# simonkosina/vbt

Hardware: AMD Instinct MI355X
Metric: frames/sec end-to-end (detect+NMS+track), EfficientDet-Lite0 320x320 (higher is better)
Workload: dtype int8

## Files before the change

### vbt_amd/csrc/band_block.h

```cpp
#pragma once
#include <type_traits>

#include "fused_block.h"

namespace vbt {

#ifndef VBT_BD_WAVES
#define VBT_BD_WAVES 16
#endif
constexpr int BD_WAVES = VBT_BD_WAVES, BD_THREADS = 64 * BD_WAVES;
constexpr int BD_LIT = 3;
constexpr int BD_LIT_NODE = 1;
constexpr int BD_LIT_NODE_WIDE = 3;
constexpr int BD_WP_TAIL = 1024;
constexpr int BD_WD_CHAIN = 12 * 1024 + 512;

#ifdef VBT_BD_PROF
#define BD_STAMP(k) do { if (threadIdx.x == 0) a.prof[(long)blockIdx.x * 8 + (k)] = __builtin_amdgcn_s_memtime(); } while (0)
#else
#define BD_STAMP(k) do { } while (0)
#endif

struct BandArgs {
  const int8_t* x;
  int8_t* out;
  int H, W, Cout, rows, nbands;
  int C, CS;
  int NCG, KS;
  unsigned zx4;
  const v4i* wd;
  const int* bd;
  const float* md;
  Rq rqd;
  const v4i* wp;
  const v4i* wpc;
  const int* bp;
  const float* mp;
  Rq rqp;
  int n_src, chain;
  const int8_t* src[3];
  int sh[3], sw[3], smode[3], spt[3], spl[3];
  AddQ sumq, preq;
#ifdef VBT_BD_PROF
  unsigned long long* prof;
#endif
};

__device__ __forceinline__ unsigned band_source4(const BandArgs& a, int j, long b, int iy, int ix, int cd, bool up2) {
  const int C = a.C;
  const int8_t* sb = a.src[j] + b * (long)a.sh[j] * a.sw[j] * C + 4 * cd;
  if (a.smode[j] == 0) return *(const unsigned*)(sb + (iy * a.sw[j] + ix) * C);
  if (a.smode[j] == 1) {
    int yy, xx;
    if (up2) { yy = iy >> 1; xx = ix >> 1; }
    else { yy = (iy * a.sh[j]) / a.H; xx = (ix * a.sw[j]) / a.W; }
    return *(const unsigned*)(sb + (yy * a.sw[j] + xx) * C);
  }
  unsigned lo = 0u, hi = 0u;
#pragma unroll
  for (int ky = 0; ky < 3; ky++) {
    const int yy = iy * 2 + ky - a.spt[j], yc = min(max(yy, 0), a.sh[j] - 1);
#pragma unroll
    for (int kx = 0; kx < 3; kx++) {
      const int xx = ix * 2 + kx - a.spl[j], xc = min(max(xx, 0), a.sw[j] - 1);
      unsigned t = *(const unsigned*)(sb + (yc * a.sw[j] + xc) * C);
      t = (yy == yc && xx == xc) ? (t ^ 0x80808080u) : 0u;
      lo = pk_max_u16(lo, t & 0x00FF00FFu);
      hi = pk_max_u16(hi, (t >> 8) & 0x00FF00FFu);
    }
  }
  return (lo | (hi << 8)) ^ 0x80808080u;
}

__device__ __forceinline__ uint4 band_source16(const BandArgs& a, int j, long b, int iy, int ix, int sg, bool up2) {
  const int C = a.C;
  const int8_t* sb = a.src[j] + b * (long)a.sh[j] * a.sw[j] * C + 16 * sg;
  if (a.smode[j] == 0) return *(const uint4*)(sb + (iy * a.sw[j] + ix) * C);
  if (a.smode[j] == 1) {
    int yy, xx;
    if (up2) { yy = iy >> 1; xx = ix >> 1; }
    else { yy = (iy * a.sh[j]) / a.H; xx = (ix * a.sw[j]) / a.W; }
    return *(const uint4*)(sb + (yy * a.sw[j] + xx) * C);
  }
  unsigned lo[4] = {0u, 0u, 0u, 0u}, hi[4] = {0u, 0u, 0u, 0u};
#pragma unroll
  for (int ky = 0; ky < 3; ky++) {
    const int yy = iy * 2 + ky - a.spt[j], yc = min(max(yy, 0), a.sh[j] - 1);
#pragma unroll
    for (int kx = 0; kx < 3; kx++) {
      const int xx = ix * 2 + kx - a.spl[j], xc = min(max(xx, 0), a.sw[j] - 1);
      const uint4 t4 = *(const uint4*)(sb + (yc * a.sw[j] + xc) * C);
      const bool in = yy == yc && xx == xc;
      const unsigned tt[4] = {t4.x, t4.y, t4.z, t4.w};
#pragma unroll
      for (int d = 0; d < 4; d++) {
        const unsigned t = in ? (tt[d] ^ 0x80808080u) : 0u;
        lo[d] = pk_max_u16(lo[d], t & 0x00FF00FFu);
        hi[d] = pk_max_u16(hi[d], (t >> 8) & 0x00FF00FFu);
      }
    }
  }
  return make_uint4((lo[0] | (hi[0] << 8)) ^ 0x80808080u, (lo[1] | (hi[1] << 8)) ^ 0x80808080u, (lo[2] | (hi[2] << 8)) ^ 0x80808080u,
                    (lo[3] | (hi[3] << 8)) ^ 0x80808080u);
}

template <int NW, int CT, bool NODES = true, bool CHAIN = false>
__device__ __forceinline__ void sepconv_band_body(const BandArgs& a, int local, unsigned char* bd_smem) {
  constexpr int nwaves = NW, nthreads = 64 * NW;
  static_assert(!CHAIN || CT == 64, "the chained form is built for 64-channel maps");
  constexpr bool C64 = CT == 64, CK = CT != 0;
  constexpr int CS_T = CT == 64 ? 80 : CT;
  static_assert(CT == 0 || CT == 64 || CT == 112, "compile-time widths: 64, 112");
  const long b = fdiv_small(local, frcp(a.nbands));
  const int band = local - (int)b * a.nbands;
  const int tid = threadIdx.x, wave = tid >> 6, lane = tid & 63, r = lane & 15, g = lane >> 4;
  const int y0 = band * a.rows, nr = min(a.rows, a.H - y0);
  const int PW = a.W + 2, NPh = (nr + 2) * PW, NPo = nr * a.W, NPG = (NPo + 15) >> 4;
  const int C = CK ? CT : a.C, CS = CK ? CS_T : a.CS;
  unsigned char* T0 = bd_smem;
  unsigned char* D = T0 + (a.rows + 2) * PW * CS;
  unsigned char* WP = CHAIN ? D : D + (((a.rows * a.W + 15) >> 4) << 4) * CS;
  const int NT = (a.Cout + 15) >> 4, KS = CK ? (CT + 63) / 64 : a.KS, NCG = CK ? (CT + 15) / 16 : a.NCG;
  unsigned char* WB = WP + NT * KS * 1024;
  BD_STAMP(0);

  const v4i* wpg = CHAIN ? a.wpc : a.wp;
  for (int i = tid; i < NT * KS * 64; i += nthreads) *(v4i*)(WP + 16 * i) = wpg[i];
  if constexpr (CHAIN) {
    for (int i = tid; i < 12 * 64; i += nthreads) *(v4i*)(WB + BD_WP_TAIL + 16 * i) = a.wd[i];
    if (tid >= 64 && tid < 80) *(uint4*)(WB + BD_WP_TAIL + 12 * 1024 + 16 * (tid - 64)) = *(const uint4*)((const unsigned char*)a.bd + 16 * (tid - 64));
    else if (tid >= 96 && tid < 112) *(uint4*)(WB + BD_WP_TAIL + 12 * 1024 + 256 + 16 * (tid - 96)) = *(const uint4*)((const unsigned char*)a.md + 16 * (tid - 96));
  }
  if (tid < 4 * NT) *(uint4*)(WB + 16 * tid) = *(const uint4*)((const unsigned char*)a.bp + 16 * tid);
  else if (tid >= 32 && tid < 32 + 4 * NT) *(uint4*)(WB + 512 + 16 * (tid - 32)) = *(const uint4*)((const unsigned char*)a.mp + 16 * (tid - 32));
  const float rcp_pw = frcp(PW);
  if (NODES && a.n_src > 0) {
    const bool up2[3] = {a.H == 2 * a.sh[0] && a.W == 2 * a.sw[0], a.H == 2 * a.sh[1] && a.W == 2 * a.sw[1], a.H == 2 * a.sh[2] && a.W == 2 * a.sw[2]};
    if (CK || (C & 15) == 0) {
      constexpr int LITN = C64 ? BD_LIT_NODE : BD_LIT_NODE_WIDE;
      const int npp = C64 ? 4 : CS >> 4, nreal = C64 ? 4 : C >> 4;
      const float rcp_npp = frcp(npp);
      const int total = NPh * npp;
      for (int i0 = tid; i0 < total; i0 += LITN * nthreads) {
        uint4 us[LITN][3];
        int pofs[LITN];
#pragma unroll
        for (int k = 0; k < LITN; k++) {
          const int i = i0 + k * nthreads, ic = min(i, total - 1);
          const int p = C64 ? ic >> 2 : (CK ? ic / (CS_T >> 4) : fdiv_small(ic, rcp_npp)), sg = ic - p * npp;
          const int hy = fdiv_small(p, rcp_pw), hx = p - hy * PW;
          const int iy = y0 + hy - 1, ix = hx - 1;
          const bool in = i < total && sg < nreal && iy >= 0 && iy < a.H && ix >= 0 && ix < a.W;
          pofs[k] = i < total ? (p * CS + 16 * sg) | (in ? 0 : (1 << 30)) : -1;
#pragma unroll
          for (int j = 0; j < 3; j++) {
            us[k][j] = make_uint4(0u, 0u, 0u, 0u);
            if (j < a.n_src && in) us[k][j] = band_source16(a, j, b, iy, ix, sg, up2[j]);
          }
        }
#pragma unroll
        for (int k = 0; k < LITN; k++) {
          if (pofs[k] < 0) continue;
          uint4 v = make_uint4(a.zx4, a.zx4, a.zx4, a.zx4);
          if (!(pofs[k] >> 30)) {
            const unsigned u0[4] = {us[k][0].x, us[k][0].y, us[k][0].z, us[k][0].w}, u1[4] = {us[k][1].x, us[k][1].y, us[k][1].z, us[k][1].w},
                           u2[4] = {us[k][2].x, us[k][2].y, us[k][2].z, us[k][2].w};
            unsigned o[4];
#pragma unroll
            for (int d = 0; d < 4; d++) {
              if (a.chain == 0) o[d] = addq4(u0[d], u1[d], a.sumq);
              else {
                const unsigned pp = addq4(u0[d], u1[d], a.preq);
                o[d] = a.chain == 1 ? addq4(pp, u2[d], a.sumq) : addq4(u2[d], pp, a.sumq);
              }
            }
            v = make_uint4(o[0], o[1], o[2], o[3]);
          }
          *(uint4*)(T0 + (pofs[k] & 0xFFFFFF)) = v;
        }
      }
    } else {
    const int ndp = CS >> 2, nd = C >> 2;
    const float rcp_ndp = frcp(ndp);
    for (int i = tid; i < NPh * ndp; i += nthreads) {
      const int p = fdiv_small(i, rcp_ndp), cd = i - p * ndp;
      const int hy = fdiv_small(p, rcp_pw), hx = p - hy * PW;
      const int iy = y0 + hy - 1, ix = hx - 1;
      unsigned v = a.zx4;
      if (cd < nd && iy >= 0 && iy < a.H && ix >= 0 && ix < a.W) {
        unsigned us[3] = {0u, 0u, 0u};
#pragma unroll
        for (int j = 0; j < 3; j++)
          if (j < a.n_src) us[j] = band_source4(a, j, b, iy, ix, cd, up2[j]);
        if (a.chain == 0) v = addq4(us[0], us[1], a.sumq);
        else {
          const unsigned pp = addq4(us[0], us[1], a.preq);
          v = a.chain == 1 ? addq4(pp, us[2], a.sumq) : addq4(us[2], pp, a.sumq);
        }
      }
      *(unsigned*)(T0 + p * CS + 4 * cd) = v;
    }
    }
  } else {
    const int8_t* xb = a.x + b * (long)a.H * a.W * C;
    if constexpr (C64) {
      const uint4 z4 = make_uint4(a.zx4, a.zx4, a.zx4, a.zx4);
      const int total = NPh * 4;
      for (int i0 = tid; i0 < total; i0 += BD_LIT * nthreads) {
        uint4 v[BD_LIT];
        int pofs[BD_LIT];
#pragma unroll
        for (int k = 0; k < BD_LIT; k++) {
          const int i = i0 + k * nthreads;
          const int p = i >> 2, sg = i & 3;
          const int hy = fdiv_small(min(p, NPh - 1), rcp_pw), hx = p - hy * PW;
          const int iy = y0 + hy - 1, ix = hx - 1;
          pofs[k] = i < total ? p * 80 + 16 * sg : -1;
          v[k] = z4;
          if (i < total && iy >= 0 && iy < a.H && ix >= 0 && ix < a.W) v[k] = *(const uint4*)(xb + (iy * a.W + ix) * 64 + 16 * sg);
        }
#pragma unroll
        for (int k = 0; k < BD_LIT; k++)
          if (pofs[k] >= 0) *(uint4*)(T0 + pofs[k]) = v[k];
      }
    } else {
    if (CK || (C & 15) == 0) {
      const int npp = CS >> 4, nreal = C >> 4;
      const float rcp_npp = frcp(npp);
      const uint4 z4 = make_uint4(a.zx4, a.zx4, a.zx4, a.zx4);
      const int total = NPh * npp;
      for (int i0 = tid; i0 < total; i0 += BD_LIT * nthreads) {
        uint4 v[BD_LIT];
        int pofs[BD_LIT];
#pragma unroll
        for (int k = 0; k < BD_LIT; k++) {
          const int i = i0 + k * nthreads, ic = min(i, total - 1);
          const int p = CK ? ic / (CS_T >> 4) : fdiv_small(ic, rcp_npp), sg = ic - p * npp;
          const int hy = fdiv_small(p, rcp_pw), hx = p - hy * PW;
          const int iy = y0 + hy - 1, ix = hx - 1;
          pofs[k] = i < total ? p * CS + 16 * sg : -1;
          v[k] = z4;
          if (i < total && sg < nreal && iy >= 0 && iy < a.H && ix >= 0 && ix < a.W) v[k] = *(const uint4*)(xb + (iy * a.W + ix) * C + 16 * sg);
        }
#pragma unroll
        for (int k = 0; k < BD_LIT; k++)
          if (pofs[k] >= 0) *(uint4*)(T0 + pofs[k]) = v[k];
      }
    } else {
    const int ngp = CS >> 3, ng = C >> 3;
    const float rcp_ngp = frcp(ngp);
    const uint2 z2 = make_uint2(a.zx4, a.zx4);
    for (int i = tid; i < NPh * ngp; i += nthreads) {
      const int p = fdiv_small(i, rcp_ngp), sg = i - p * ngp;
      const int hy = fdiv_small(p, rcp_pw), hx = p - hy * PW;
      const int iy = y0 + hy - 1, ix = hx - 1;
      uint2 v = z2;
      if (sg < ng && iy >= 0 && iy < a.H && ix >= 0 && ix < a.W) v = *(const uint2*)(xb + (iy * a.W + ix) * C + 8 * sg);
      *(uint2*)(T0 + p * CS + 8 * sg) = v;
    }
    }
    }
  }
  int tapoff[3];
#pragma unroll
  for (int m = 0; m < 3; m++) {
    const int tap = min(4 * m + g, 8);
    tapoff[m] = ((tap / 3) * PW + (tap % 3)) * CS;
  }
  const float rcp_w = frcp(a.W);
  if constexpr (CHAIN) {
    const unsigned char* WD = WB + BD_WP_TAIL;
    const unsigned char* WDB = WD + 12 * 1024;
    __syncthreads();
    BD_STAMP(1);
    int8_t* ob = a.out + ((b * a.H + y0) * (long)a.W) * a.Cout + 4 * g;
    const bool dword_out = (a.Cout & 3) == 0;
    auto chain = [&](auto fd_c, auto u_c, int pg0) {
      constexpr int U = decltype(u_c)::value, FULL = decltype(fd_c)::value;
      int slot[U];
      const unsigned char* pb[U];
#pragma unroll
      for (int u = 0; u < U; u++) {
        slot[u] = (pg0 + u * nwaves) * 16 + r;
        const int sc = min(slot[u], NPo - 1);
        const int py = fdiv_small(sc, rcp_w);
        pb[u] = T0 + (sc + 2 * py) * CS;
      }
      v4i dv[U];
      {
#pragma unroll
        for (int cg = 0; cg < 4; cg++) {
          v4i wdv[3], bv[U][3], acc[U];
#pragma unroll
          for (int m = 0; m < 3; m++) wdv[m] = *(const v4i*)(WD + ((cg * 3 + m) * 64 + lane) * 16);
          const int4 bq = *(const int4*)(WDB + 64 * cg + 16 * g);
          const float4 mu = *(const float4*)(WDB + 256 + 64 * cg + 16 * g);
#pragma unroll
          for (int u = 0; u < U; u++)
#pragma unroll
            for (int m = 0; m < 3; m++) bv[u][m] = *(const v4i*)(pb[u] + tapoff[m] + 16 * cg);
#pragma unroll
          for (int u = 0; u < U; u++) acc[u] = v4i_from(int4_plus(bq, FULL >= 2 ? RQ_KBIAS : 0));
#pragma unroll
          for (int m = 0; m < 3; m++)
#pragma unroll
            for (int u = 0; u < U; u++) acc[u] = __builtin_amdgcn_mfma_i32_16x16x64_i8(wdv[m], bv[u][m], acc[u], 0, 0, 0);
#pragma unroll
          for (int u = 0; u < U; u++) dv[u][cg] = (int)rq_pack_b<FULL>(acc[u], mu, a.rqd);
          __builtin_amdgcn_sched_barrier(0);
        }
      }
      rq_dispatch(a.rqp, [&](auto fp_c) {
        constexpr int FULL = decltype(fp_c)::value;
        for (int t = 0; t < NT; t++) {
          const int c0 = 16 * t + 4 * g;
          const v4i wv = *(const v4i*)(WP + (t * 64 + lane) * 16);
          const int4 bb = *(const int4*)(WB + 4 * c0);
          const float4 mm = *(const float4*)(WB + 512 + 4 * c0);
          v4i acc[U];
#pragma unroll
          for (int u = 0; u < U; u++) acc[u] = __builtin_amdgcn_mfma_i32_16x16x64_i8(wv, dv[u], v4i_from(int4_plus(bb, FULL >= 2 ? RQ_KBIAS : 0)), 0, 0, 0);
#pragma unroll
          for (int u = 0; u < U; u++) {
            const unsigned d = rq_pack_b<FULL>(acc[u], mm, a.rqp);
            if (slot[u] < NPo && c0 < a.Cout) {
              int8_t* o = ob + (long)slot[u] * a.Cout + 16 * t;
              if (dword_out) *(unsigned*)o = d;
              else
                for (int j = 0; j < 4; j++)
                  if (c0 + j < a.Cout) o[j] = (int8_t)(d >> (8 * j));
            }
          }
        }
      });
    };
    rq_dispatch(a.rqd, [&](auto fd_c) {
      int pg = wave;
      for (; pg + nwaves < NPG; pg += 2 * nwaves) chain(fd_c, std::integral_constant<int, 2>{}, pg);
      if (pg < NPG) chain(fd_c, std::integral_constant<int, 1>{}, pg);
    });
    BD_STAMP(3);
    return;
  }
  const int cg = wave % NCG, sub = wave / NCG, nsub = nwaves / NCG;
  v4i wdv[3];
#pragma unroll
  for (int m = 0; m < 3; m++) wdv[m] = a.wd[(cg * 3 + m) * 64 + lane];
  const int4 bq = *(const int4*)(a.bd + 16 * cg + 4 * g);
  const float4 mu = *(const float4*)(a.md + 16 * cg + 4 * g);
  __syncthreads();
  BD_STAMP(1);
  if (sub < nsub) {
    auto d_units = [&](auto full_c, auto u_c, int pg0) {
      constexpr int U = decltype(u_c)::value, FULL = decltype(full_c)::value;
      const unsigned char* pb[U];
      int slot[U];
#pragma unroll
      for (int u = 0; u < U; u++) {
        slot[u] = (pg0 + u * nsub) * 16 + r;
        const int sc = min(slot[u], NPo - 1);
        const int py = fdiv_small(sc, rcp_w);
        pb[u] = T0 + (sc + 2 * py) * CS + 16 * cg;
      }
      v4i bv[U][3], acc[U];
#pragma unroll
      for (int u = 0; u < U; u++)
#pragma unroll
        for (int m = 0; m < 3; m++) bv[u][m] = *(const v4i*)(pb[u] + tapoff[m]);
#pragma unroll
      for (int u = 0; u < U; u++) acc[u] = v4i_from(int4_plus(bq, FULL >= 2 ? RQ_KBIAS : 0));
#pragma unroll
      for (int m = 0; m < 3; m++)
#pragma unroll
        for (int u = 0; u < U; u++) acc[u] = __builtin_amdgcn_mfma_i32_16x16x64_i8(wdv[m], bv[u][m], acc[u], 0, 0, 0);
#pragma unroll
      for (int u = 0; u < U; u++) *(unsigned*)(D + slot[u] * CS + 16 * cg + 4 * g) = rq_pack_b<FULL>(acc[u], mu, a.rqd);
    };
    auto d_walk = [&](auto full_c) {
      int pg = sub;
      for (; pg + nsub < NPG; pg += 2 * nsub) d_units(full_c, std::integral_constant<int, 2>{}, pg);
      if (pg < NPG) d_units(full_c, std::integral_constant<int, 1>{}, pg);
    };
    rq_dispatch(a.rqd, d_walk);
  }
  __syncthreads();
  BD_STAMP(2);
  const int NU = NPG * NT;
  const float rcp_nt = frcp(NT);
  auto store_unit = [&](int pg, int t, const v4i& acc, const float4& mm) {
    const int slot = pg * 16 + r;
    const int c0 = 16 * t + 4 * g;
    const unsigned d = rq_pack_b(acc, mm, a.rqp);
    if (slot < NPo && c0 < a.Cout) {
      int8_t* o = a.out + ((b * a.H + y0) * (long)a.W + slot) * a.Cout + c0;
      if ((a.Cout & 3) == 0) *(unsigned*)o = d;
      else
        for (int j = 0; j < 4; j++)
          if (c0 + j < a.Cout) o[j] = (int8_t)(d >> (8 * j));
    }
  };
  if (NT == 4 && KS == 1 && a.Cout == 64) {
    const int t = wave & 3, c0 = 16 * t + 4 * g;
    const v4i wv = *(const v4i*)(WP + (t * 64 + lane) * 16);
    const int4 bb = *(const int4*)(WB + 4 * c0);
    const float4 mm = *(const float4*)(WB + 512 + 4 * c0);
    int8_t* ob = a.out + ((b * a.H + y0) * (long)a.W) * a.Cout + c0;
    auto p_units = [&](auto full_c, auto u_c, int pg0) {
      constexpr int U = decltype(u_c)::value, FULL = decltype(full_c)::value;
      v4i dv[U], acc[U];
#pragma unroll
      for (int u = 0; u < U; u++) dv[u] = *(const v4i*)(D + ((pg0 + u * (nwaves / 4)) * 16 + r) * CS + 16 * g);
#pragma unroll
      for (int u = 0; u < U; u++) acc[u] = __builtin_amdgcn_mfma_i32_16x16x64_i8(wv, dv[u], v4i_from(int4_plus(bb, FULL >= 2 ? RQ_KBIAS : 0)), 0, 0, 0);
#pragma unroll
      for (int u = 0; u < U; u++) {
        const int slot = (pg0 + u * (nwaves / 4)) * 16 + r;
        const unsigned d = rq_pack_b<FULL>(acc[u], mm, a.rqp);
        if (slot < NPo) *(unsigned*)(ob + (long)slot * a.Cout) = d;
      }
    };
    auto p_walk = [&](auto full_c) {
      int pg = wave >> 2;
      for (; pg + (nwaves / 4) < NPG; pg += 2 * (nwaves / 4)) p_units(full_c, std::integral_constant<int, 2>{}, pg);
      if (pg < NPG) p_units(full_c, std::integral_constant<int, 1>{}, pg);
    };
    rq_dispatch(a.rqp, p_walk);
  } else if (!C64 && NT <= nwaves && KS <= 2 && (nwaves - NT * (nwaves / NT)) * 8 <= nwaves) {
    const int t = wave % NT, sub = wave / NT, nsub = nwaves / NT;
    if (sub < nsub) {
      const int c0 = 16 * t + 4 * g;
      v4i wv[2];
#pragma unroll
      for (int ks = 0; ks < 2; ks++) wv[ks] = ks < KS ? *(const v4i*)(WP + ((t * KS + ks) * 64 + lane) * 16) : (v4i){0, 0, 0, 0};
      const int4 bb = *(const int4*)(WB + 4 * c0);
      const float4 mm = *(const float4*)(WB + 512 + 4 * c0);
      auto p_units = [&](auto u_c, int pg0) {
        constexpr int U = decltype(u_c)::value;
        v4i dv[U][2], acc[U];
#pragma unroll
        for (int u = 0; u < U; u++)
#pragma unroll
          for (int ks = 0; ks < 2; ks++)
            if (ks < KS) dv[u][ks] = *(const v4i*)(D + ((pg0 + u * nsub) * 16 + r) * CS + 16 * g + 64 * ks);
#pragma unroll
        for (int u = 0; u < U; u++) {
          acc[u] = __builtin_amdgcn_mfma_i32_16x16x64_i8(wv[0], dv[u][0], v4i_from(bb), 0, 0, 0);
          if (KS > 1) acc[u] = __builtin_amdgcn_mfma_i32_16x16x64_i8(wv[1], dv[u][1], acc[u], 0, 0, 0);
        }
#pragma unroll
        for (int u = 0; u < U; u++) store_unit(pg0 + u * nsub, t, acc[u], mm);
      };
      int pg = sub;
      for (; pg + nsub < NPG; pg += 2 * nsub) p_units(std::integral_constant<int, 2>{}, pg);
      if (pg < NPG) p_units(std::integral_constant<int, 1>{}, pg);
    }
  } else {
    for (int u = wave; u < NU; u += nwaves) {
      const int pg = fdiv_small(u, rcp_nt), t = u - pg * NT;
      const int c0 = 16 * t + 4 * g;
      v4i acc = v4i_from(*(const int4*)(WB + 4 * c0));
      const unsigned char* drow = D + (pg * 16 + r) * CS + 16 * g;
      for (int ks = 0; ks < KS; ks++)
        acc = __builtin_amdgcn_mfma_i32_16x16x64_i8(*(const v4i*)(WP + ((t * KS + ks) * 64 + lane) * 16), *(const v4i*)(drow + 64 * ks), acc, 0, 0, 0);
      store_unit(pg, t, acc, *(const float4*)(WB + 512 + 4 * c0));
    }
  }
  BD_STAMP(3);
}

#ifndef VBT_BD_HEAD_WAVES
#define VBT_BD_HEAD_WAVES 8
#endif
#ifndef VBT_BD_HEAD_MAXPX
#define VBT_BD_HEAD_MAXPX 240
#endif
constexpr int BD_HEAD_WAVES = VBT_BD_HEAD_WAVES, BD_HEAD_MAXPX = VBT_BD_HEAD_MAXPX;
constexpr int BD_HEAD_WAVES_WIDE = 16;
#ifdef VBT_DEFINE_BAND_KERNELS
__device__ __forceinline__ int band_problem(const MultiTiles& mt) {
  int pi = 0;
#pragma unroll
  for (int i = 1; i < 12; i++)
    if (i < mt.n && (int)blockIdx.x >= mt.start[i]) pi = i;
  return pi;
}
__global__ __launch_bounds__(64 * BD_HEAD_WAVES) void sepconv_band_kernel(const BandArgs* __restrict__ probs, MultiTiles mt) {
  extern __shared__ __attribute__((aligned(16))) unsigned char bd_smem_dyn[];
  const int pi = band_problem(mt);
  sepconv_band_body<BD_HEAD_WAVES, 64, false>(probs[pi], (int)blockIdx.x - mt.start[pi], bd_smem_dyn);
}
__global__ __launch_bounds__(64 * BD_HEAD_WAVES_WIDE, 2) void sepconv_band_wide_kernel(const BandArgs* __restrict__ probs, MultiTiles mt) {
  extern __shared__ __attribute__((aligned(16))) unsigned char bd_smem_dyn[];
  const int pi = band_problem(mt);
  sepconv_band_body<BD_HEAD_WAVES_WIDE, 0, false>(probs[pi], (int)blockIdx.x - mt.start[pi], bd_smem_dyn);
}
__global__ __launch_bounds__(64 * BD_HEAD_WAVES_WIDE, 2) void sepconv_band_c112_kernel(const BandArgs* __restrict__ probs, MultiTiles mt) {
  extern __shared__ __attribute__((aligned(16))) unsigned char bd_smem_dyn[];
  const int pi = band_problem(mt);
  sepconv_band_body<BD_HEAD_WAVES_WIDE, 112, false>(probs[pi], (int)blockIdx.x - mt.start[pi], bd_smem_dyn);
}
__global__ __launch_bounds__(64 * BD_HEAD_WAVES) __attribute__((amdgpu_waves_per_eu(6))) void sepconv_band_chain_kernel(const BandArgs* __restrict__ probs, MultiTiles mt) {
  extern __shared__ __attribute__((aligned(16))) unsigned char bd_smem_dyn[];
  const int pi = band_problem(mt);
  sepconv_band_body<BD_HEAD_WAVES, 64, false, true>(probs[pi], (int)blockIdx.x - mt.start[pi], bd_smem_dyn);
}
__global__ __launch_bounds__(BD_THREADS) void sepconv_band_one_kernel(BandArgs a) {
  extern __shared__ __attribute__((aligned(16))) unsigned char bd_smem_dyn[];
  sepconv_band_body<BD_WAVES, 64>(a, (int)blockIdx.x, bd_smem_dyn);
}
__global__ __launch_bounds__(BD_THREADS) void sepconv_band_one_chain_kernel(BandArgs a) {
  extern __shared__ __attribute__((aligned(16))) unsigned char bd_smem_dyn[];
  sepconv_band_body<BD_WAVES, 64, true, true>(a, (int)blockIdx.x, bd_smem_dyn);
}
__global__ __launch_bounds__(BD_THREADS) void sepconv_band_one_wide_kernel(BandArgs a) {
  extern __shared__ __attribute__((aligned(16))) unsigned char bd_smem_dyn[];
  sepconv_band_body<BD_WAVES, 0>(a, (int)blockIdx.x, bd_smem_dyn);
}
__global__ __launch_bounds__(BD_THREADS) void sepconv_band_one_c112_kernel(BandArgs a) {
  extern __shared__ __attribute__((aligned(16))) unsigned char bd_smem_dyn[];
  sepconv_band_body<BD_WAVES, 112>(a, (int)blockIdx.x, bd_smem_dyn);
}
#endif

}
```

### vbt_amd/csrc/dev_common.h

```cpp
#pragma once
#include "common.h"

namespace vbt {

typedef int v4i __attribute__((ext_vector_type(4)));

__device__ __forceinline__ int requant(int acc, float mult, int zp, int lo, int hi) {
  float t = (float)acc * mult;
  t = fminf(fmaxf(t, -65536.0f), 65536.0f);
  int q = (int)__builtin_rintf(t) + zp;
  return min(max(q, lo), hi);
}
__device__ __forceinline__ unsigned pack4(int a, int b, int c, int d) {
  return (unsigned)(a & 255) | ((unsigned)(b & 255) << 8) | ((unsigned)(c & 255) << 16) | ((unsigned)(d & 255) << 24);
}

struct Rq {
  float lo_f, hi_f, off;
  int full;
  int kb;
};
constexpr int RQ_KBIAS = 0x4B400000;
__host__ __device__ inline Rq make_rq(int zp, int lo, int hi, int kb = 0) {
  return Rq{(float)(lo - zp), (float)(hi - zp), (float)(zp + 128), (lo <= -128 && hi >= 127) ? 1 : 0, kb};
}
__device__ __forceinline__ float rq_u8(float accf, float mult, const Rq& q) {
  float r = __builtin_rintf(accf * mult);
  return __builtin_amdgcn_fmed3f(r, q.lo_f, q.hi_f) + q.off;
}
__device__ __forceinline__ unsigned pack4_u8f(float a, float b, float c, float d) {
  unsigned v = __builtin_amdgcn_cvt_pk_u8_f32(a, 0, 0);
  v = __builtin_amdgcn_cvt_pk_u8_f32(b, 1, v);
  v = __builtin_amdgcn_cvt_pk_u8_f32(c, 2, v);
  v = __builtin_amdgcn_cvt_pk_u8_f32(d, 3, v);
  return v ^ 0x80808080u;
}
typedef float v2f __attribute__((ext_vector_type(2)));
template <int FULLK = -1>
__device__ __forceinline__ unsigned rq_pack_b(const v4i& acc, const float4& mu, const Rq& q) {
  v2f f0, f1;
  if (FULLK >= 2) {
    const v2f kf = {12582912.0f, 12582912.0f};
    f0 = (v2f){__int_as_float(acc[0]), __int_as_float(acc[1])} - kf;
    f1 = (v2f){__int_as_float(acc[2]), __int_as_float(acc[3])} - kf;
  } else {
    f0 = (v2f){(float)acc[0], (float)acc[1]};
    f1 = (v2f){(float)acc[2], (float)acc[3]};
  }
  v2f t0 = f0 * (v2f){mu.x, mu.y};
  v2f t1 = f1 * (v2f){mu.z, mu.w};
  const v2f off = {q.off, q.off};
  if ((FULLK >= 0 && (FULLK & 1)) || (FULLK < 0 && q.full)) {
    const v2f magic = {12582912.0f, 12582912.0f};
    const v2f back = {q.off - 12582912.0f, q.off - 12582912.0f};
    v2f r0 = (t0 + magic) + back;
    v2f r1 = (t1 + magic) + back;
    return pack4_u8f(r0.x, r0.y, r1.x, r1.y);
  }
  v2f r0 = {__builtin_amdgcn_fmed3f(__builtin_rintf(t0.x), q.lo_f, q.hi_f), __builtin_amdgcn_fmed3f(__builtin_rintf(t0.y), q.lo_f, q.hi_f)};
  v2f r1 = {__builtin_amdgcn_fmed3f(__builtin_rintf(t1.x), q.lo_f, q.hi_f), __builtin_amdgcn_fmed3f(__builtin_rintf(t1.y), q.lo_f, q.hi_f)};
  r0 = r0 + off;
  r1 = r1 + off;
  return pack4_u8f(r0.x, r0.y, r1.x, r1.y);
}
__device__ __forceinline__ v4i diag_operand(unsigned wb, int i) {
  const unsigned sh = wb << (8 * (i & 3));
  const int d = i >> 2;
  return (v4i){d == 0 ? (int)sh : 0, d == 1 ? (int)sh : 0, d == 2 ? (int)sh : 0, d == 3 ? (int)sh : 0};
}
__device__ __forceinline__ v4i toeplitz_operand(unsigned w4, int c) {
  const int sh = 8 * c;
  return (v4i){(int)((w4 & 0xffu) << sh), (int)(((w4 >> 8) & 0xffu) << sh), (int)(((w4 >> 16) & 0xffu) << sh), (int)((w4 >> 24) << sh)};
}
__device__ __forceinline__ int fdiv_small(int n, float rcp_d) { return (int)(((float)n + 0.5f) * rcp_d); }
__device__ __forceinline__ float frcp(int d) { return __builtin_amdgcn_rcpf((float)d); }
__device__ __forceinline__ v4i v4i_from(const int4& b) { return (v4i){b.x, b.y, b.z, b.w}; }
__device__ __forceinline__ int4 int4_plus(const int4& b, int k) { return make_int4(b.x + k, b.y + k, b.z + k, b.w + k); }
template <class F>
__device__ __forceinline__ void rq_dispatch(const Rq& q, F&& f) {
  if (q.kb) { if (q.full) f(std::integral_constant<int, 3>{}); else f(std::integral_constant<int, 2>{}); }
  else { if (q.full) f(std::integral_constant<int, 1>{}); else f(std::integral_constant<int, 0>{}); }
}

__device__ __forceinline__ unsigned rq_pack_i(const v4i& acc, const int4& b, const float4& mu, const Rq& q) {
  const v4i a2 = {acc[0] + b.x, acc[1] + b.y, acc[2] + b.z, acc[3] + b.w};
  return rq_pack_b(a2, mu, q);
}

struct AddQ { int bias, am, bm, shift, lo, hi, off; };
static inline AddQ make_addq(const AddParams& p, int z_out, int lo, int hi) {
  return AddQ{p.bias, p.am, p.bm, p.shift, lo - z_out, hi - z_out, z_out + 128};
}
__device__ __forceinline__ int addq_u8(int a, int b, const AddQ& q) {
  const int t = (q.bias + __mul24(a, q.am) + __mul24(b, q.bm)) >> q.shift;
  return min(max(t, q.lo), q.hi) + q.off;
}
__device__ __forceinline__ unsigned addq4(unsigned ua, unsigned ub, const AddQ& q) {
  unsigned r = 0;
#pragma unroll
  for (int e = 0; e < 4; e++)
    r |= (unsigned)addq_u8((int)(int8_t)(ua >> (8 * e)), (int)(int8_t)(ub >> (8 * e)), q) << (8 * e);
  return r ^ 0x80808080u;
}

__device__ __forceinline__ unsigned max4_s8(unsigned a, unsigned b) {
  unsigned r = 0;
#pragma unroll
  for (int j = 0; j < 4; j++) {
    int x = (int)(int8_t)(a >> (8 * j)), y = (int)(int8_t)(b >> (8 * j));
    r |= (unsigned)(max(x, y) & 255) << (8 * j);
  }
  return r;
}

struct Epi {
  const int* bias;
  const float* mult;
  int zp, lo, hi;
  Rq rq;
};

__device__ __forceinline__ void store_tile(const v4i acc[4], const Epi& e, int8_t* __restrict__ out, long m, int N,
                                           int nb, int g) {
  int c0 = nb * 64 + 16 * g;
  if (c0 >= N) return;
  unsigned d[4];
#pragma unroll
  for (int t = 0; t < 4; t++) {
    int4 b = *(const int4*)(e.bias + c0 + 4 * t);
    float4 mu = *(const float4*)(e.mult + c0 + 4 * t);
    d[t] = rq_pack_i(acc[t], b, mu, e.rq);
  }
  int8_t* o = out + m * N + c0;
  if ((N & 15) == 0) {
    *(uint4*)o = make_uint4(d[0], d[1], d[2], d[3]);
  } else if ((N & 3) == 0) {
#pragma unroll
    for (int t = 0; t < 4; t++)
      if (c0 + 4 * t < N) *(unsigned*)(o + 4 * t) = d[t];
  } else {
#pragma unroll
    for (int t = 0; t < 4; t++)
#pragma unroll
      for (int j = 0; j < 4; j++)
        if (c0 + 4 * t + j < N) o[4 * t + j] = (int8_t)(d[t] >> (8 * j));
  }
}

}
```

### vbt_amd/csrc/fused_block.h

```cpp
#pragma once
#include "tpz_geom.h"
#include "halo_geom.h"
#include "fused_params_geom.h"
#include "dev_common.h"

namespace vbt {

struct FusedArgs {
  const int8_t* x;
  int8_t* out;
  int H, W, Cin, OH, OW, Cout;
  int pad_t, pad_l;
  int TX, TY, tiles_x, tiles_y;
  int T0S;
  int nchunks;
  int zx;
  const long* we;
  const int* be;
  const float* me;
  int KSe, ze, loe, hie;
  Rq rqe;
  const long* we3;
  const long* wdm3;
  const v4i* wp3;
  int nch3, KSp3;
  const float* wd;
  const int* bd;
  const float* md;
  int zd, lod, hid;
  Rq rqd;
  const long* wdm;
  const int* bdm;
  const v4i* wd64;
  const long* wd64c;
  const unsigned* wtz;
  const v4i* wp;
  const v4i* wpt;
  const v4i* wpt3;
  const int* bp;
  const float* mp;
  int KSp, zo, lop, hip;
  Rq rqp;
  const unsigned char* cpar;
  int has_res;
  AddQ resq;
  int n_src;
  const int8_t* src[3];
  int sh[3], sw[3], smode[3], spt[3], spl[3];
  int chain;
  AddQ sumq, preq;
};

__device__ __forceinline__ unsigned node_sum4(const unsigned u[3], const FusedArgs& a) {
  if (a.chain == 0) return addq4(u[0], u[1], a.sumq);
  const unsigned p = addq4(u[0], u[1], a.preq);
  return a.chain == 1 ? addq4(p, u[2], a.sumq) : addq4(u[2], p, a.sumq);
}

typedef unsigned short v2u16 __attribute__((ext_vector_type(2)));
__device__ __forceinline__ unsigned pk_max_u16(unsigned a, unsigned b) {
  v2u16 x, y;
  __builtin_memcpy(&x, &a, 4);
  __builtin_memcpy(&y, &b, 4);
  v2u16 r = __builtin_elementwise_max(x, y);
  unsigned o;
  __builtin_memcpy(&o, &r, 4);
  return o;
}

constexpr int FB_EST = 80;
constexpr int FB_DST = 80;

template <int NP> struct ParamPieces { v4i v[NP > 0 ? (NP + 255) / 256 : 1]; };
template <int NP> __device__ __forceinline__ void pp_fetch(ParamPieces<NP>& r, const unsigned char* src, int tid) {
#pragma unroll
  for (int i = 0; i < (NP + 255) / 256; i++) r.v[i] = *(const v4i*)(src + 16 * min(tid + 256 * i, NP - 1));
}
template <int NP> __device__ __forceinline__ void pp_store(const ParamPieces<NP>& r, unsigned char* dst, int tid) {
#pragma unroll
  for (int i = 0; i < (NP + 255) / 256; i++)
    if (256 * i + 255 < NP || tid + 256 * i < NP) *(v4i*)(dst + 16 * (tid + 256 * i)) = r.v[i];
}
template <int KK, int S, int NBP, bool EXPAND, bool MDW, int KSE = 0, int NT = 4, int PPW = 1, bool DW64 = false, bool TPZ = false, int NTL = 0, bool PLDS = false>
__device__ __forceinline__ void fused_block_body(const FusedArgs& a, int tile, unsigned char* fb_smem) {
  static_assert(PPW == 1 || MDW, "128-pixel tiles exist for the matrix-pipe depthwise only");
  static_assert(NTL >= 0 && NTL <= 4 && (NTL == 0 || EXPAND), "a tile-major last block (MBConv only) holds one to four tiles");
  constexpr int NBW = NTL ? NBP - 1 : NBP;
  static_assert(!DW64 || (EXPAND && MDW && (KK == 3 || KK == 5)), "DW64: fused expand blocks, 3x3 / 5x5");
  static_assert(!TPZ || (DW64 && (S == 1 || S == 2) && (NT == 3 || NT == 4) && NBP <= 2 && (KSE == 1 || KSE == 2)), "TPZ: a form of DW64");
  constexpr TpzGeom TG = TPZ ? tpz_geom(KK, S, PPW, NT) : TpzGeom{};
  constexpr int KT2 = (S * (S - 1) + KK + 1) / 2;
  static_assert(!PLDS || (EXPAND && MDW && (KSE == 1 || KSE == 2)), "PLDS: MBConv tiles with register-resident expand weights and no early depthwise request");
  constexpr FusedParamsGeom PG = fused_params_geom(NT, KSE > 0 ? KSE : 1, TPZ ? FPF_TOEPLITZ : DW64 ? FPF_DIAG64 : FPF_MATRIX, KK, S, NBP, NTL);
  constexpr int NPE = PLDS ? PG.pe / 16 : 0, NPD = PLDS ? PG.pd / 16 : 0, NPP = PLDS ? PG.pp / 16 : 0, NPB = PLDS ? PG.pb / 16 : 0;
  const int tid = threadIdx.x, wave = __builtin_amdgcn_readfirstlane(tid >> 6), lane = tid & 63, r = lane & 15, g = lane >> 4;
  const int trow = fdiv_small(tile, frcp(a.tiles_x));
  const int tx = tile - trow * a.tiles_x;
  const int bimg = fdiv_small(trow, frcp(a.tiles_y));
  const int ty = trow - bimg * a.tiles_y;
  const long b = bimg;
  const int oy0 = ty * a.TY, ox0 = tx * a.TX;
  const int TXp = (a.TX + 3) & ~3;
  const int HWx = (TXp - 1) * S + KK, HWy = (a.TY - 1) * S + KK, NPh = HWx * HWy;
  const int iy0 = oy0 * S - a.pad_t, ix0 = ox0 * S - a.pad_l;
  const float rcp_hwx = frcp(HWx), rcp_txp = frcp(TXp);
  unsigned char* T0 = fb_smem;
  unsigned char* E = T0 + ((NPh * a.T0S + 15) & ~15);
  constexpr int EST = (EXPAND && NT == 3) ? (DW64 ? 48 : 72) : FB_EST;
  unsigned char* D = E + (EXPAND ? (TPZ ? TG.e_bytes : ((NPh * EST + 15) & ~15)) : 0);
  bool stage_p = false;
  if constexpr (!EXPAND && NBP <= 2) stage_p = a.nchunks == 1;
  unsigned char* WPS = D + 64 * PPW * FB_DST;
  unsigned char* BPS = WPS + NBP * 4096;
  unsigned char* const PAe = D + 64 * PPW * FB_DST + (TPZ ? 8 * TG.DSK : 0);
  unsigned char* const PAd = PAe + PG.pe;
  unsigned char* const PAp = PAd + PG.pd;
  unsigned char* const PAb = PAp + PG.pp;
  constexpr int CH = 16 * NT;
  const int nch = NT == 3 ? a.nch3 : a.nchunks;
  ParamPieces<NPE> rpe;
  ParamPieces<NPD> rpd;
  ParamPieces<NPP> rpp;
  ParamPieces<NPB> rpb;
  if constexpr (PLDS) {
    pp_fetch(rpe, a.cpar, tid);
    pp_fetch(rpd, a.cpar + PG.pe, tid);
    pp_fetch(rpp, a.cpar + PG.pe + PG.pd, tid);
    pp_fetch(rpb, a.cpar + (long)nch * PG.chunk, tid);
  }

  bool summed = false;
  if constexpr (!EXPAND) summed = a.n_src > 0;
  if (summed) {
    const int nd = a.Cin >> 2;
    const unsigned zb4 = (unsigned)(a.zx & 255) * 0x01010101u;
    const int pstep = fdiv_small(256, frcp(nd));
    int p = fdiv_small(tid, frcp(nd));
    const int cd = tid - p * nd;
    const bool up2[3] = {a.H == 2 * a.sh[0] && a.W == 2 * a.sw[0], a.H == 2 * a.sh[1] && a.W == 2 * a.sw[1], a.H == 2 * a.sh[2] && a.W == 2 * a.sw[2]};
    for (; tid < pstep * nd && p < NPh; p += pstep) {
      const int hy = fdiv_small(p, rcp_hwx), hx = p - hy * HWx;
      const int iy = iy0 + hy, ix = ix0 + hx;
      unsigned v = zb4;
      if (!halo_outside(iy, ix, a.H, a.W)) {
        unsigned us[3] = {0u, 0u, 0u};
#pragma unroll
        for (int j = 0; j < 3; j++) {
          if (j < a.n_src) {
            const int8_t* sb = a.src[j] + b * (long)a.sh[j] * a.sw[j] * a.Cin + 4 * cd;
            unsigned u;
            if (a.smode[j] == 0) {
              u = *(const unsigned*)(sb + ((long)iy * a.sw[j] + ix) * a.Cin);
            } else if (a.smode[j] == 1) {
              int yy, xx;
              if (up2[j]) { yy = iy >> 1; xx = ix >> 1; }
              else { yy = (iy * a.sh[j]) / a.H; xx = (ix * a.sw[j]) / a.W; }
              u = *(const unsigned*)(sb + ((long)yy * a.sw[j] + xx) * a.Cin);
            } else {
              unsigned tv[9];
#pragma unroll
              for (int ky = 0; ky < 3; ky++) {
                const int yy = iy * 2 + ky - a.spt[j];
                const int yc = min(max(yy, 0), a.sh[j] - 1);
#pragma unroll
                for (int kx = 0; kx < 3; kx++) {
                  const int xx = ix * 2 + kx - a.spl[j];
                  const int xc = min(max(xx, 0), a.sw[j] - 1);
                  const unsigned t = *(const unsigned*)(sb + ((long)yc * a.sw[j] + xc) * a.Cin);
                  tv[ky * 3 + kx] = (yy == yc && xx == xc) ? (t ^ 0x80808080u) : 0u;
                }
              }
              unsigned lo = 0u, hi = 0u;
#pragma unroll
              for (int q = 0; q < 9; q++) {
                const unsigned l = tv[q] & 0x00FF00FFu, h = (tv[q] >> 8) & 0x00FF00FFu;
                lo = pk_max_u16(lo, l);
                hi = pk_max_u16(hi, h);
              }
              u = (lo | (hi << 8)) ^ 0x80808080u;
            }
            us[j] = u;
          }
        }
        v = node_sum4(us, a);
      }
      *(unsigned*)(T0 + p * a.T0S + 4 * cd) = v;
    }
  } else {
    if ((a.Cin & 15) == 0) {
      const int ng = a.Cin >> 4;
      const unsigned zb1 = (unsigned)(a.zx & 255) * 0x01010101u;
      const uint4 zb = make_uint4(zb1, zb1, zb1, zb1);
      const int8_t* xb = a.x + b * (long)a.H * a.W * a.Cin;
      const int pstep = fdiv_small(256, frcp(ng));
      int p = fdiv_small(tid, frcp(ng));
      const int sg = tid - p * ng;
      for (; tid < pstep * ng && p < NPh; p += pstep) {
        const int hy = fdiv_small(p, rcp_hwx), hx = p - hy * HWx;
        const int iy = iy0 + hy, ix = ix0 + hx;
        uint4 v = zb;
        if (!halo_outside(iy, ix, a.H, a.W)) v = *(const uint4*)(xb + (iy * a.W + ix) * a.Cin + 16 * sg);
        unsigned char* dst = T0 + p * a.T0S + 16 * sg;
        if constexpr (EXPAND) {
          *(uint2*)dst = make_uint2(v.x, v.y);
          *(uint2*)(dst + 8) = make_uint2(v.z, v.w);
        } else {
          *(uint4*)dst = v;
        }
      }
    } else {
    const int ng = a.Cin >> 3;
    const unsigned long long zb = (unsigned long long)(a.zx & 255) * 0x0101010101010101ull;
    const int8_t* xb = a.x + b * (long)a.H * a.W * a.Cin;
    const int pstep = fdiv_small(256, frcp(ng));
    int p = fdiv_small(tid, frcp(ng));
    const int sg = tid - p * ng;
    for (; tid < pstep * ng && p < NPh; p += pstep) {
      const int hy = fdiv_small(p, rcp_hwx), hx = p - hy * HWx;
      const int iy = iy0 + hy, ix = ix0 + hx;
      unsigned long long v = zb;
      if (!halo_outside(iy, ix, a.H, a.W)) v = *(const unsigned long long*)(xb + (iy * a.W + ix) * a.Cin + 8 * sg);
      *(unsigned long long*)(T0 + p * a.T0S + 8 * sg) = v;
    }
    }
  }
  if (stage_p) {
    for (int i = tid; i < NBP * 256; i += 256) *(uint4*)(WPS + 16 * i) = *(const uint4*)((const unsigned char*)a.wp + 16 * (long)i);
    if (tid < NBP * 16) *(uint4*)(BPS + 16 * tid) = *(const uint4*)((const unsigned char*)a.bp + 16 * tid);
    else if (tid < NBP * 32) *(uint4*)(BPS + 16 * tid) = *(const uint4*)((const unsigned char*)a.mp + 16 * (tid - NBP * 16));
  }
  const int NPG = (NPh + 15) >> 4;
  unsigned oob_mask = 0;
  const bool border = EXPAND && halo_border(iy0, ix0, HWx, HWy, a.H, a.W);
  if (border) oob_mask = halo_oob_mask(wave, r, NPh, HWx, iy0, ix0, a.H, a.W, [&](int p) { return fdiv_small(p, rcp_hwx); });
  v4i acc[PPW][NBP][4];
#pragma unroll
  for (int pp = 0; pp < PPW; pp++)
#pragma unroll
    for (int nb = 0; nb < NBP; nb++)
#pragma unroll
      for (int t = 0; t < 4; t++) acc[pp][nb][t] = (v4i){0, 0, 0, 0};
  const int cq = tid & 15, strip = tid >> 4;
  const int nsx = TXp >> 2;
  const int sy = fdiv_small(strip, frcp(nsx)), sx = (strip - sy * nsx) * 4;
  const bool dw_active = sy < a.TY;
  int hbase[4 * PPW];
#pragma unroll
  for (int pg = 0; pg < 4 * PPW; pg++) hbase[pg] = 0;
  if constexpr (MDW && !DW64) {
#pragma unroll
    for (int pg = 0; pg < 4 * PPW; pg++) {
      int slot = pg * 16 + r;
      int sq = TXp == 8 ? (slot >> 3) : fdiv_small(slot, rcp_txp);
      int py_ = min(sq, a.TY - 1), px_ = slot - sq * TXp;
      hbase[pg] = (py_ * S) * HWx + px_ * S;
    }
  }
  const int wq0 = TPZ ? wave * NT : 0;
  int tz_e = 0, tz_d = 0;
  if constexpr (TPZ) {
    tz_e = tpz_e_offset(TG, S, r, g, wq0);
    tz_d = tpz_d_offset(TG, S, PPW, FB_DST, r, g, wq0);
  }
  constexpr int KTP = (KK * KK + 1) / 2;
  long wpre[KTP];
  int4 bpre = make_int4(0, 0, 0, 0);
  float4 mpre = make_float4(0.f, 0.f, 0.f, 0.f);
  if constexpr (!EXPAND && MDW) {
    const long* wm0 = a.wdm + ((long)wave * KTP) * 64 + lane;
#pragma unroll
    for (int mi = 0; mi < KTP; mi++) wpre[mi] = wm0[mi * 64];
    bpre = *(const int4*)(a.bdm + 16 * wave + 4 * g);
    mpre = *(const float4*)(a.md + 16 * wave + 4 * g);
  }
  if constexpr (PLDS) {
    pp_store(rpe, PAe, tid);
    pp_store(rpd, PAd, tid);
    pp_store(rpp, PAp, tid);
    pp_store(rpb, PAb, tid);
  }
  __syncthreads();

  const long* const wdm_ = NT == 3 ? a.wdm3 : a.wdm;
  for (int c = 0; c < nch; c++) {
    constexpr bool PREF_DW = EXPAND && MDW && KSE >= 3;
    if constexpr (PREF_DW) {
      if (NT == 4 || wave < NT) {
        const long* wmc = wdm_ + ((long)(c * NT + wave) * KTP) * 64 + lane;
#pragma unroll
        for (int mi = 0; mi < KTP; mi++) wpre[mi] = wmc[mi * 64];
        bpre = *(const int4*)(a.bdm + c * CH + 16 * wave + 4 * g);
        mpre = *(const float4*)(a.md + c * CH + 16 * wave + 4 * g);
      }
    }
    unsigned wtz[TPZ ? NT * KT2 : 1];
    if constexpr (TPZ && !PLDS) {
      const unsigned* wt = a.wtz + ((long)(c * 4 * NT + wq0) * KT2) * 64 + lane;
#pragma unroll
      for (int i = 0; i < NT * KT2; i++) wtz[i] = wt[i * 64];
    }
    const unsigned char* const cnext = PLDS ? a.cpar + (long)min(c + 1, nch - 1) * PG.chunk : nullptr;
    if (EXPAND) {
      int4 eb[NT];
      float4 em[NT];
      const unsigned zeb = (unsigned)(a.ze & 255) * 0x01010101u;
      const long* w = (NT == 3 ? a.we3 : a.we) + (long)c * a.KSe * NT * 64 + lane;
      long wreg[KSE > 0 ? KSE : 1][NT];
      if constexpr (PLDS) {
        pp_fetch(rpe, cnext, tid);
#pragma unroll
        for (int t = 0; t < NT; t++) {
          eb[t] = *(const int4*)(PAe + PG.o_be + 4 * (4 * NT * g + 4 * t));
          em[t] = *(const float4*)(PAe + PG.o_me + 4 * (4 * NT * g + 4 * t));
        }
#pragma unroll
        for (int ks = 0; ks < KSE; ks++)
#pragma unroll
          for (int t = 0; t < NT; t++) wreg[ks][t] = *(const long*)(PAe + 8 * ((ks * NT + t) * 64 + lane));
      } else {
#pragma unroll
      for (int t = 0; t < NT; t++) {
        eb[t] = *(const int4*)(a.be + c * CH + 4 * NT * g + 4 * t);
        em[t] = *(const float4*)(a.me + c * CH + 4 * NT * g + 4 * t);
      }
      if constexpr (KSE > 0) {
#pragma unroll
        for (int ks = 0; ks < KSE; ks++)
#pragma unroll
          for (int t = 0; t < NT; t++) wreg[ks][t] = w[(ks * NT + t) * 64];
      }
      }
      auto expand_loop = [&](auto full_tag, auto oob_tag) {
        constexpr int FULLK = decltype(full_tag)::value;
        constexpr bool OOB = decltype(oob_tag)::value;
        int4 ebk[NT];
#pragma unroll
        for (int t = 0; t < NT; t++) ebk[t] = int4_plus(eb[t], FULLK >= 2 ? RQ_KBIAS : 0);
        for (int i = 0, pg = wave; pg < NPG; pg += 4, i++) {
          const int p = pg * 16 + r;
          v4i ea[NT];
#pragma unroll
          for (int t = 0; t < NT; t++) ea[t] = v4i_from(ebk[t]);
          const unsigned char* brow = T0 + (__umul24((unsigned)min(p, NPh - 1), (unsigned)a.T0S) + 8u * g);
          if constexpr (KSE > 0) {
#pragma unroll
            for (int ks = 0; ks < KSE; ks++) {
              long bv = *(const long*)(brow + 32 * ks);
#pragma unroll
              for (int t = 0; t < NT; t++) ea[t] = __builtin_amdgcn_mfma_i32_16x16x32_i8(wreg[ks][t], bv, ea[t], 0, 0, 0);
            }
          } else {
#pragma unroll 2
            for (int ks = 0; ks < a.KSe; ks++) {
              long bv = *(const long*)(brow + 32 * ks);
#pragma unroll
              for (int t = 0; t < NT; t++) ea[t] = __builtin_amdgcn_mfma_i32_16x16x32_i8(w[(ks * NT + t) * 64], bv, ea[t], 0, 0, 0);
            }
          }
          unsigned d[NT];
#pragma unroll
          for (int t = 0; t < NT; t++) {
            d[t] = rq_pack_b<FULLK>(ea[t], em[t], a.rqe);
            if constexpr (OOB)
              if ((oob_mask >> i) & 1u) d[t] = zeb;
          }
          if (p < NPh) {
            if constexpr (TPZ) {
              const int hy = fdiv_small(p, rcp_hwx), hx = p - hy * HWx;
              unsigned char* ep = E + tpz_e_store(TG, hy, hx, NT * g);
#pragma unroll
              for (int t = 0; t < NT; t++) *(unsigned*)(ep + t * TG.EQS) = d[t];
            } else if constexpr (NT == 4) {
              *(uint4*)(E + p * FB_EST + 16 * g) = make_uint4(d[0], d[1], d[2], d[3]);
            } else {
#pragma unroll
              for (int t = 0; t < NT; t++) *(unsigned*)(E + p * EST + 4 * NT * g + 4 * t) = d[t];
            }
          }
        }
      };
      if (border) rq_dispatch(a.rqe, [&](auto full_tag) { expand_loop(full_tag, std::true_type{}); });
      else rq_dispatch(a.rqe, [&](auto full_tag) { expand_loop(full_tag, std::false_type{}); });
      __syncthreads();
      if constexpr (PLDS) {
        pp_store(rpe, PAe, tid);
        if (c > 0) pp_store(rpp, PAp, tid);
        pp_fetch(rpd, cnext + PG.pe, tid);
      }
    }
    if constexpr (TPZ) {
      constexpr int NU = NT * PPW, PGE = tpz_e_group(TG, S), PGD = tpz_d_group(TG, PPW, FB_DST);
      int4 bq[NT];
      float4 mq[NT];
      if constexpr (!PLDS) {
#pragma unroll
        for (int q = 0; q < NT; q++) {
          bq[q] = *(const int4*)(a.bdm + c * CH + 4 * (wq0 + q));
          mq[q] = *(const float4*)(a.md + c * CH + 4 * (wq0 + q));
        }
      }
      const unsigned char* const tzw = PAd + 4 * (wq0 * KT2 * 64 + lane);
      const unsigned char* const tzb = PAd + 16 * wq0;
      auto tz_bias = [&](int q) { if constexpr (PLDS) return *(const int4*)(tzb + PG.o_bd + 16 * q); else return bq[q]; };
      auto tz_mult = [&](int q) { if constexpr (PLDS) return *(const float4*)(tzb + PG.o_md + 16 * q); else return mq[q]; };
      auto tz_tap = [&](int i) { if constexpr (PLDS) return *(const unsigned*)(tzw + 256 * i); else return wtz[i]; };
      const unsigned char* eb = E + tz_e;
      unsigned char* db = D + tz_d;
      auto tz_walk = [&](auto mode_tag) {
        constexpr int RM = decltype(mode_tag)::value;
#pragma unroll
        for (int u0 = 0; u0 < NU; u0 += 2) {
          v4i dq[2];
#pragma unroll
          for (int u = 0; u < 2; u++) dq[u] = v4i_from(int4_plus(tz_bias((u0 + u < NU ? u0 + u : u0) / PPW), RM >= 2 ? RQ_KBIAS : 0));
#pragma unroll
          for (int mi = 0; mi < KT2; mi++)
#pragma unroll
            for (int u = 0; u < 2; u++) {
              if (u0 + u >= NU) continue;
              const int q = (u0 + u) / PPW, pg = (u0 + u) % PPW;
              const v4i bv = *(const v4i*)(eb + q * TG.EQS + pg * PGE + mi * 2 * TG.EYS);
              dq[u] = __builtin_amdgcn_mfma_i32_16x16x64_i8(toeplitz_operand(tz_tap(q * KT2 + mi), r & 3), bv, dq[u], 0, 0, 0);
            }
#pragma unroll
          for (int u = 0; u < 2; u++) {
            if (u0 + u >= NU) continue;
            const int q = (u0 + u) / PPW, pg = (u0 + u) % PPW;
            *(unsigned*)(db + pg * PGD + 4 * q) = rq_pack_b<RM>(dq[u], tz_mult(q), a.rqd);
          }
        }
      };
      rq_dispatch(a.rqd, tz_walk);
    } else if constexpr (DW64) {
      constexpr int TXP = 8 * PPW, HWX = (TXP - 1) * S + KK;
      constexpr int KT64 = KK == 3 ? 3 : 7;
      constexpr int PGS = (16 / TXP) * S * HWX * EST;
      if (NT == 4 || wave < NT) {
        const unsigned long long wc = PLDS ? *(const unsigned long long*)(PAd + 8 * (wave * 64 + lane)) : (unsigned long long)a.wd64c[(long)(c * NT + wave) * 64 + lane];
        v4i wreg[KT64];
#pragma unroll
        for (int mi = 0; mi < KT64; mi++) wreg[mi] = diag_operand((unsigned)(wc >> (8 * mi)) & 0xffu, r);
        const int4 bq0 = PLDS ? *(const int4*)(PAd + PG.o_bd + 4 * (16 * wave + 4 * g)) : *(const int4*)(a.bdm + c * CH + 16 * wave + 4 * g);
        const float4 mum = PLDS ? *(const float4*)(PAd + PG.o_md + 4 * (16 * wave + 4 * g)) : *(const float4*)(a.md + c * CH + 16 * wave + 4 * g);
        const int hb = TXP == 8 ? ((r >> 3) * S * HWX + (r & 7) * S) : r * S;
        const unsigned char* baseH = E + hb * EST + 16 * wave + g * EST;
        const unsigned char* baseV = E + hb * EST + 16 * wave + g * (HWX * EST);
        auto dw_walk = [&](auto mode_tag) {
          constexpr int RM = decltype(mode_tag)::value;
          const int4 bqm = int4_plus(bq0, RM >= 2 ? RQ_KBIAS : 0);
#pragma unroll
          for (int pg = 0; pg < 4 * PPW; pg += 2) {
            v4i dqa = v4i_from(bqm), dqb = v4i_from(bqm);
#pragma unroll
            for (int mi = 0; mi < KT64; mi++) {
              const unsigned char* bp = (KK == 5 && mi == 5) ? baseV : baseH;
              const int off = KK == 3 ? mi * HWX * EST : (mi < 5 ? mi * HWX * EST : (mi == 5 ? 4 * EST : (4 * HWX + 4) * EST));
              const v4i bva = *(const v4i*)(bp + pg * PGS + off);
              const v4i bvb = *(const v4i*)(bp + (pg + 1) * PGS + off);
              dqa = __builtin_amdgcn_mfma_i32_16x16x64_i8(wreg[mi], bva, dqa, 0, 0, 0);
              dqb = __builtin_amdgcn_mfma_i32_16x16x64_i8(wreg[mi], bvb, dqb, 0, 0, 0);
            }
            *(unsigned*)(D + (pg * 16 + r) * FB_DST + 16 * wave + 4 * g) = rq_pack_b<RM>(dqa, mum, a.rqd);
            *(unsigned*)(D + ((pg + 1) * 16 + r) * FB_DST + 16 * wave + 4 * g) = rq_pack_b<RM>(dqb, mum, a.rqd);
          }
        };
        rq_dispatch(a.rqd, dw_walk);
      }
    } else if constexpr (MDW) {
      constexpr int KT = (KK * KK + 1) / 2;
      const unsigned char* Ein = EXPAND ? E : T0 + 64 * c;
      const int est = EXPAND ? EST : a.T0S;
// ... 349 lines not shown
```

### vbt_amd/csrc/k_postprocess.hip

```cpp
#include "launchers.h"

namespace vbt {

constexpr int POST_CAP = 2048;
#ifdef VBT_POST_PROF
__device__ unsigned long long g_post_prof[16];
#define POST_STAMP(i) do { if (threadIdx.x == 0 && blockIdx.x == 0) { const unsigned long long t_ = __builtin_amdgcn_s_memtime(); atomicAdd(&g_post_prof[i], t_ - t_last); t_last = t_; } } while (0)
#else
#define POST_STAMP(i) do { } while (0)
#endif

constexpr int POST_THREADS = 1024;
constexpr int POST_FAST = 1024;
constexpr int POST_LDS_FIXED = 32768 + 1024 + 1024 + 2048 + 2048 + 256 + 32 * 16 + 128 + 128;
static_assert(POST_CAP * 4 + POST_FAST * 4 + POST_FAST * 16 + POST_FAST * 4 <= 32768, "keys | sorted keys | boxes | scores share the histogram's 32 KB");
int post_lds_bytes(int A) { return ((A + 15) & ~15) + POST_LDS_FIXED; }

__device__ __forceinline__ int wave_incl_scan_i(int x) {
  x += __builtin_amdgcn_update_dpp(0, x, 0x111, 0xf, 0xf, false);
  x += __builtin_amdgcn_update_dpp(0, x, 0x112, 0xf, 0xf, false);
  x += __builtin_amdgcn_update_dpp(0, x, 0x114, 0xf, 0xf, false);
  x += __builtin_amdgcn_update_dpp(0, x, 0x118, 0xf, 0xf, false);
  x += __builtin_amdgcn_update_dpp(0, x, 0x142, 0xa, 0xf, false);
  x += __builtin_amdgcn_update_dpp(0, x, 0x143, 0xc, 0xf, false);
  return x;
}
__device__ __forceinline__ int wave_first_lane(bool flag) {
  const unsigned long long m = __ballot(flag);
  return m ? __ffsll((long long)m) - 1 : 64;
}

__global__ __launch_bounds__(POST_THREADS) void postprocess_kernel(PostArgs p, float* __restrict__ boxes, float* __restrict__ scores,
                                                                   float* __restrict__ classes, int* __restrict__ counts) {
  extern __shared__ __attribute__((aligned(16))) unsigned char post_smem[];
  constexpr int NT = POST_THREADS;
  const int tid = threadIdx.x, lane = tid & 63, wave = tid >> 6;
  const long b = blockIdx.x;
#ifdef VBT_POST_PROF
  unsigned long long t_last = __builtin_amdgcn_s_memtime();
#endif
  const int A = p.A;
  int* hist32 = (int*)post_smem;
  unsigned* keys = (unsigned*)hist32;
  unsigned* skeys = keys + POST_CAP;
  float4* lbox = (float4*)(skeys + POST_FAST);
  float* lsc = (float*)(lbox + POST_FAST);
  int* rhist = (int*)(post_smem + 32768);
  float* s_score = (float*)(rhist + 256);
  double* s_dq = (double*)(s_score + 256);
  double* s_ex = s_dq + 256;
  signed char* s_rank = (signed char*)(s_ex + 256);
  float4* selbox = (float4*)(s_rank + 256);
  int* sv = (int*)(selbox + 32);
  unsigned char* cb = post_smem + POST_LDS_FIXED;
  int& s_n = sv[0]; int& s_qlo = sv[1]; int& s_qhi = sv[2]; int& s_i0 = sv[3]; int& s_i1 = sv[4]; int& s_nsel = sv[5]; int& s_done = sv[6];
  int& s_blo = sv[7]; int& s_bhi = sv[8];
  int* s_wtot = sv + 12;
  constexpr int PS = 5;
  const int n4 = (A + 3) >> 2;
  const int b1 = p.base[1], b2 = p.base[2], b3 = p.base[3], b4 = p.base[4];
  auto level_of = [&](int a) -> int { return (a >= b1) + (a >= b2) + (a >= b3) + (a >= b4); };
  const unsigned char *pc0, *pb0;
  long ce1, ce2, ce3, ce4, be1, be2, be3, be4;
  {
    auto cbias = [&](int l) { return (long)p.cls[l] + (b * (long)(p.base[l + 1] - p.base[l]) - p.base[l]) * (long)p.C; };
    auto bbias = [&](int l) { return (long)p.box[l] + (b * (long)(p.base[l + 1] - p.base[l]) - p.base[l]) * 4; };
    pc0 = (const unsigned char*)cbias(0); pb0 = (const unsigned char*)bbias(0);
    ce1 = cbias(1) - cbias(0); ce2 = cbias(2) - cbias(1); ce3 = cbias(3) - cbias(2); ce4 = cbias(4) - cbias(3);
    be1 = bbias(1) - bbias(0); be2 = bbias(2) - bbias(1); be3 = bbias(3) - bbias(2); be4 = bbias(4) - bbias(3);
  }
  auto cls_ptr = [&](int a) -> const unsigned char* {
    long o = (long)a * p.C;
    o += a >= b1 ? ce1 : 0l; o += a >= b2 ? ce2 : 0l; o += a >= b3 ? ce3 : 0l; o += a >= b4 ? ce4 : 0l;
    return pc0 + o;
  };
  auto box_ptr = [&](int a) -> const unsigned char* {
    long o = 4l * a;
    o += a >= b1 ? be1 : 0l; o += a >= b2 ? be2 : 0l; o += a >= b3 ? be3 : 0l; o += a >= b4 ? be4 : 0l;
    return pb0 + o;
  };
  auto whole = [&](int i, const unsigned char* src) -> bool {
    const int a = 4 * i;
    return level_of(a) == level_of(a + 3) && a + 3 < A && (((unsigned long)src) & 3ul) == 0;
  };
  auto patch = [&](int i) -> unsigned {
    unsigned w = 0;
    for (int e = 0; e < 4; e++)
      if (4 * i + e < A) w |= (unsigned)*cls_ptr(4 * i + e) << (8 * e);
    return w;
  };
  if (p.C == 1) {
    unsigned w[PS];
#pragma unroll
    for (int k = 0; k < PS; k++)
      w[k] = *(const unsigned*)((unsigned long)cls_ptr(4 * min(tid + NT * k, n4 - 1)) & ~3ul);
#pragma unroll
    for (int k = 0; k < PS; k++)
      if (tid + NT * k < n4) ((unsigned*)cb)[tid + NT * k] = w[k];
#pragma unroll 1
    for (int i = tid + NT * PS; i < n4; i += NT) ((unsigned*)cb)[i] = *(const unsigned*)((unsigned long)cls_ptr(4 * i) & ~3ul);
#pragma unroll 1
    for (int i = tid; i < n4; i += NT)
      if (!whole(i, cls_ptr(4 * i))) ((unsigned*)cb)[i] = patch(i);
  } else {
    auto best4 = [&](int i) -> unsigned {
      unsigned w = 0;
#pragma unroll
      for (int e = 0; e < 4; e++) {
        const int a = min(4 * i + e, A - 1);
        const signed char* src = (const signed char*)cls_ptr(a);
        int best = src[0];
        for (int c = 1; c < p.C; c++) best = max(best, (int)src[c]);
        w |= ((unsigned)best & 255u) << (8 * e);
      }
      return w;
    };
    if (p.C == 2) {
      constexpr unsigned HB = 0x80808080u;
      auto pair_max = [&](uint2 v) -> unsigned {
        const unsigned w0 = v.x ^ HB, w1 = v.y ^ HB;
        const unsigned m0 = pk_max_u16(w0 & 0x00FF00FFu, (w0 >> 8) & 0x00FF00FFu);
        const unsigned m1 = pk_max_u16(w1 & 0x00FF00FFu, (w1 >> 8) & 0x00FF00FFu);
        return ((m0 & 0xFFu) | ((m0 >> 8) & 0xFF00u) | ((m1 & 0xFFu) << 16) | ((m1 << 8) & 0xFF000000u)) ^ HB;
      };
      auto whole2 = [&](int i, const unsigned char* src) -> bool {
        const int a = 4 * i;
        return level_of(a) == level_of(a + 3) && a + 3 < A && (((unsigned long)src) & 7ul) == 0;
      };
      uint2 w[PS];
#pragma unroll
      for (int k = 0; k < PS; k++)
        w[k] = *(const uint2*)((unsigned long)cls_ptr(4 * min(tid + NT * k, n4 - 1)) & ~7ul);
#pragma unroll
      for (int k = 0; k < PS; k++)
        if (tid + NT * k < n4) ((unsigned*)cb)[tid + NT * k] = pair_max(w[k]);
#pragma unroll 1
      for (int i = tid + NT * PS; i < n4; i += NT) ((unsigned*)cb)[i] = pair_max(*(const uint2*)((unsigned long)cls_ptr(4 * i) & ~7ul));
#pragma unroll 1
      for (int i = tid; i < n4; i += NT)
        if (!whole2(i, cls_ptr(4 * i))) ((unsigned*)cb)[i] = best4(i);
    } else {
#pragma unroll 1
      for (int i = tid; i < n4; i += NT) ((unsigned*)cb)[i] = best4(i);
    }
  }
#pragma unroll
  for (int k = 0; k < 8; k++) hist32[tid + NT * k] = 0;
  if (tid < 256) {
    rhist[tid] = 0;
    s_score[tid] = ((const float*)p.tables)[tid];
    s_dq[tid] = ((const double*)(p.tables + 1024))[tid];
    s_ex[tid] = ((const double*)(p.tables + 3072))[tid];
    s_rank[tid] = ((const signed char*)(p.tables + 5120))[tid];
  }
  if (tid == 0) { s_nsel = 0; s_done = 0; }
  __syncthreads();
  POST_STAMP(0);
  unsigned u[PS];
#pragma unroll
  for (int k = 0; k < PS; k++) u[k] = ((const unsigned*)cb)[min(tid + NT * k, n4 - 1)] ^ 0x80808080u;
  {
    const int copy = tid & 31;
#pragma unroll
    for (int k = 0; k < PS; k++) {
      const int i = tid + NT * k;
#pragma unroll
      for (int e = 0; e < 4; e++)
        if (4 * i + e < A) atomicAdd(&hist32[(((u[k] >> (8 * e)) & 255u) << 5) + copy], 1);
    }
    for (int i = tid + NT * PS; i < n4; i += NT) {
      const unsigned w = ((const unsigned*)cb)[i] ^ 0x80808080u;
#pragma unroll
      for (int e = 0; e < 4; e++)
        if (4 * i + e < A) atomicAdd(&hist32[(((w >> (8 * e)) & 255u) << 5) + copy], 1);
    }
  }
  __syncthreads();
  {
    const int bin = tid >> 2, part = tid & 3;
    int c = 0;
#pragma unroll
    for (int k = 0; k < 8; k++) c += hist32[(bin << 5) + 8 * part + ((k + bin) & 7)];
    if (c) atomicAdd(&rhist[(int)s_rank[bin] + 128], c);
  }
  __syncthreads();
  POST_STAMP(1);
  int qcur = 127;
  int seg0 = 0;
  while (true) {
    if (wave == 0) {
      int v[4], before[4];
      int sum = 0;
#pragma unroll
      for (int j = 0; j < 4; j++) {
        const int r = 127 - (4 * lane + j);
        v[j] = (r <= qcur && r >= p.qmin) ? rhist[r + 128] : 0;
        before[j] = sum;
        sum += v[j];
      }
      const int excl = wave_incl_scan_i(sum) - sum;
      int ffail = 4, ftop = 4;
#pragma unroll
      for (int j = 3; j >= 0; j--) {
        const int r = 127 - (4 * lane + j);
        const int bf = excl + before[j];
        const bool ok = r > qcur || (r >= p.qmin && bf < 256 && bf + v[j] <= POST_CAP);
        if (!ok) ffail = j;
        if (v[j] > 0) ftop = j;
      }
      const int lf = wave_first_lane(ffail < 4), lt = wave_first_lane(ftop < 4);
      const int tfail = lf < 64 ? 4 * lf + __builtin_amdgcn_readlane(ffail, lf) : 256;
      const int ttop = lt < 64 ? 4 * lt + __builtin_amdgcn_readlane(ftop, lt) : 256;
      if (lane == 0) {
        if (ttop >= 256) {
          s_done = 1;
        } else if (tfail <= ttop) {
          s_qhi = 127 - ttop; s_qlo = 127 - ttop; s_i0 = seg0; s_i1 = min(seg0 + POST_CAP, A);
        } else {
          s_qhi = 127 - ttop; s_qlo = 128 - tfail; s_i0 = 0; s_i1 = A;
        }
        s_blo = 255; s_bhi = 0;
      }
    }
    __syncthreads();
    POST_STAMP(2);
    if (s_done) break;
    const int qhi = s_qhi, qlo = s_qlo, i0 = s_i0, i1 = s_i1;
    if (tid < 256) {
      const int r = (int)s_rank[tid];
      const unsigned long long m = __ballot(r >= qlo && r <= qhi);
      if (lane == 0 && m) {
        atomicMin(&s_blo, 64 * wave + __ffsll((long long)m) - 1);
        atomicMax(&s_bhi, 64 * wave + 63 - __clzll((long long)m));
      }
    }
    __syncthreads();
    POST_STAMP(11);
    {
      constexpr unsigned H = 0x80808080u;
      const unsigned LO7 = ((unsigned)s_blo * 0x01010101u) & ~H, NLO = ~((unsigned)s_blo * 0x01010101u);
      const unsigned SP = (unsigned)(s_bhi - s_blo) * 0x01010101u;
      const bool fullrange = i0 == 0 && i1 == A;
      auto hits = [&](unsigned x, int i) -> unsigned {
        const unsigned d = ((x | H) - LO7) ^ ((x ^ NLO) & H);
        const unsigned t = (SP | H) - (d & ~H);
        unsigned m = ((SP & ~d) | (~(SP ^ d) & t)) & H;
        if (fullrange) {
          if (i == n4 - 1 && (A & 3)) m &= (1u << (8 * (A & 3))) - 1u;
        } else {
          const int lo = min(max(i0 - 4 * i, 0), 4), hi = min(max(i1 - 4 * i, 0), 4);
          m &= (unsigned)(((1ull << (8 * hi)) - 1ull) & ~((1ull << (8 * lo)) - 1ull));
        }
        return m;
      };
      unsigned hm[PS];
      int cnt = 0;
#pragma unroll
      for (int k = 0; k < PS; k++) {
        hm[k] = tid + NT * k < n4 ? hits(u[k], tid + NT * k) : 0u;
        cnt += __popc(hm[k]);
      }
#pragma unroll 1
      for (int i = tid + NT * PS; i < n4; i += NT) cnt += __popc(hits(((const unsigned*)cb)[i] ^ H, i));
      const int incl = wave_incl_scan_i(cnt);
      if (lane == 63) s_wtot[wave] = incl;
      __syncthreads();
      POST_STAMP(12);
      int pos = incl - cnt;
#pragma unroll
      for (int w = 0; w < NT / 64; w++) pos += (w < wave) ? s_wtot[w] : 0;
      if (tid == NT - 1) s_n = pos + cnt;
      auto emit = [&](unsigned x, unsigned m, int i) {
#pragma unroll 1
        while (m) {
          const int e = (__ffs((int)m) - 1) >> 3;
          m &= m - 1u;
          keys[pos++] = ((unsigned)(127 - (int)s_rank[(x >> (8 * e)) & 255u]) << 16) | (unsigned)(4 * i + e);
        }
      };
#pragma unroll
      for (int k = 0; k < PS; k++)
        if (hm[k]) emit(u[k], hm[k], tid + NT * k);
#pragma unroll 1
      for (int i = tid + NT * PS; i < n4; i += NT) {
        const unsigned x = ((const unsigned*)cb)[i] ^ H;
        const unsigned m = hits(x, i);
        if (m) emit(x, m, i);
      }
    }
    __syncthreads();
    const int n = s_n;
    const bool fast = n <= POST_FAST;
    const unsigned* sk = fast ? skeys : keys;
    if (fast) {
      const int nq = (n + 3) >> 2;
      if (tid < 4 * nq - n) keys[n + tid] = 0xFFFFFFFFu;
    } else {
      int n2 = 2048;
      for (int i = n + tid; i < n2; i += NT) keys[i] = 0xFFFFFFFFu;
    }
    __syncthreads();
    POST_STAMP(3);
    if (fast) {
      const int nq = (n + 3) >> 2;
      const int parts = n > 0 ? min(NT / n, 4) : 1;
      int* partial = (int*)lbox;
      if (tid < parts * n) {
        const int m = tid % n, part = tid / n;
        const unsigned mine = keys[m];
        int r = 0;
#pragma unroll 4
        for (int j = part * nq / parts; j < (part + 1) * nq / parts; j++) {
          const uint4 k4 = ((const uint4*)keys)[j];
          r += (k4.x < mine) + (k4.y < mine) + (k4.z < mine) + (k4.w < mine);
        }
        partial[part * POST_FAST + m] = r;
      }
      __syncthreads();
      if (tid < n) {
        int r = partial[tid];
        for (int q = 1; q < parts; q++) r += partial[q * POST_FAST + tid];
        skeys[r] = keys[tid];
      }
      __syncthreads();
    } else {
      const int n2 = 2048;
      for (int k = 2; k <= n2; k <<= 1)
        for (int j = k >> 1; j > 0; j >>= 1) {
          for (int i = tid; i < n2; i += NT) {
            int ixj = i ^ j;
            if (ixj > i) {
              unsigned a = keys[i], c = keys[ixj];
              bool up = (i & k) == 0;
              if ((a > c) == up) { keys[i] = c; keys[ixj] = a; }
            }
          }
          __syncthreads();
        }
    }
    POST_STAMP(4);
#ifdef VBT_POST_PROF
    if (tid == 0 && blockIdx.x == 0) { atomicAdd(&g_post_prof[8], 1ull); atomicAdd(&g_post_prof[9], (unsigned long long)n); }
#endif
    auto decode = [&](unsigned key, float& sc) -> float4 {
      const int a = (int)(key & 0xFFFFu);
      const int q = 127 - (int)(key >> 16);
      const unsigned bq = *(const unsigned*)box_ptr(a);
      const float4 an = *(const float4*)(p.anchors + (long)a * 4);
      const float yc = (float)(s_dq[(int)((bq & 255u) ^ 128u)] * (double)an.z + (double)an.x);
      const float xc = (float)(s_dq[(int)(((bq >> 8) & 255u) ^ 128u)] * (double)an.w + (double)an.y);
      const float hh = (float)(0.5 * s_ex[(int)(((bq >> 16) & 255u) ^ 128u)] * (double)an.z);
      const float hw = (float)(0.5 * s_ex[(int)((bq >> 24) ^ 128u)] * (double)an.w);
      sc = s_score[q + 128];
      return make_float4(yc - hh, xc - hw, yc + hh, xc + hw);
    };
    if (fast) {
      if (tid < n) {
        float sc;
        lbox[tid] = decode(skeys[tid], sc);
        lsc[tid] = sc;
      }
      __syncthreads();
    }
    POST_STAMP(13);
    if (wave == 0) {
      float* selarea = (float*)(sv + 32);
      auto sup = [&](float4 sb, float sa, float4 cx, float ca) -> bool {
        const float iy0 = fmaxf(sb.x, cx.x), ix0 = fmaxf(sb.y, cx.y);
        const float iy1 = fminf(sb.z, cx.z), ix1 = fminf(sb.w, cx.w);
        const float inter = fmaxf(iy1 - iy0, 0.0f) * fmaxf(ix1 - ix0, 0.0f);
        return sa > 0.0f && ca > 0.0f && inter / (sa + ca - inter) > p.iou_thr;
      };
      int nsel = s_nsel;
      for (int base = 0; base < n && nsel < p.max_det; base += 64) {
        int ci = base + lane;
        bool alive = ci < n;
        float4 bx = make_float4(0.f, 0.f, 0.f, 0.f);
        float sc = 0.f;
        int anchor = 0;
        if (alive) {
          anchor = (int)(sk[ci] & 0xFFFFu);
          if (fast) { bx = lbox[ci]; sc = lsc[ci]; }
          else bx = decode(sk[ci], sc);
        }
        const float area = (bx.z - bx.x) * (bx.w - bx.y);
        if (alive)
          for (int s = 0; s < nsel; s++)
            if (sup(selbox[s], selarea[s], bx, area)) { alive = false; break; }
        while (nsel < p.max_det) {
          const unsigned long long mask = __ballot(alive);
          if (mask == 0ull) break;
          const int j = __ffsll((long long)mask) - 1;
          float4 sb;
          sb.x = __int_as_float(__builtin_amdgcn_readlane(__float_as_int(bx.x), j));
          sb.y = __int_as_float(__builtin_amdgcn_readlane(__float_as_int(bx.y), j));
          sb.z = __int_as_float(__builtin_amdgcn_readlane(__float_as_int(bx.z), j));
          sb.w = __int_as_float(__builtin_amdgcn_readlane(__float_as_int(bx.w), j));
          const float ss = __int_as_float(__builtin_amdgcn_readlane(__float_as_int(sc), j));
          const float sa = __int_as_float(__builtin_amdgcn_readlane(__float_as_int(area), j));
          const int sel_anchor = __builtin_amdgcn_readlane(anchor, j);
          if (lane == 0) {
            selbox[nsel] = sb;
            selarea[nsel] = sa;
            float* bo = boxes + (b * p.max_det + nsel) * 4;
            bo[0] = sb.x; bo[1] = sb.y; bo[2] = sb.z; bo[3] = sb.w;
            scores[b * p.max_det + nsel] = ss;
            int cls_id = 0;
            if (p.C > 1) {
              const unsigned char* src = cls_ptr(sel_anchor);
              int best = -128;
              for (int c = 0; c < p.C; c++) {
                const int r = (int)s_rank[(int)(src[c] ^ 128u)];
                if (r > best) { best = r; cls_id = c; }
              }
            }
            classes[b * p.max_det + nsel] = (float)cls_id;
          }
          __threadfence_block();
          nsel++;
          if (lane == j) alive = false;
          else if (alive && sup(sb, sa, bx, area)) alive = false;
        }
      }
      if (lane == 0) s_nsel = nsel;
    }
    __syncthreads();
    POST_STAMP(5);
    if (s_nsel >= p.max_det) break;
    if (qhi == qlo && rhist[qhi + 128] > POST_CAP && i1 < A) { seg0 = i1; qcur = qhi; }
    else { seg0 = 0; qcur = qlo - 1; }
    __syncthreads();
  }
  const int nsel = s_nsel;
  for (int s = nsel + tid; s < p.max_det; s += NT) {
    float* bo = boxes + (b * p.max_det + s) * 4;
    bo[0] = bo[1] = bo[2] = bo[3] = 0.0f;
    scores[b * p.max_det + s] = 0.0f;
    classes[b * p.max_det + s] = 0.0f;
  }
  if (tid == 0) counts[b] = nsel;
  POST_STAMP(6);
#ifdef VBT_POST_PROF
  if (tid == 0 && blockIdx.x == 0) atomicAdd(&g_post_prof[10], 1ull);
#endif
}

int launch_postprocess(const PostArgs& p, int lds_bytes, int B, float* boxes, float* scores, float* classes, int* counts, hipStream_t st) {
  if (lds_bytes > 64 * 1024) VBT_LDS_OPT_IN(postprocess_kernel);
  postprocess_kernel<<<dim3((unsigned)B), POST_THREADS, lds_bytes, st>>>(p, boxes, scores, classes, counts);
  return VBT_OK;
}

}

#ifdef VBT_POST_PROF
extern "C" int vbt_post_prof_read(unsigned long long* out16, int reset) {
  if (reset) { unsigned long long z[16] = {0}; VBT_HIP_CHECK(hipMemcpyToSymbol(HIP_SYMBOL(vbt::g_post_prof), z, sizeof(z))); return VBT_OK; }
  VBT_HIP_CHECK(hipDeviceSynchronize());
  VBT_HIP_CHECK(hipMemcpyFromSymbol(out16, HIP_SYMBOL(vbt::g_post_prof), 16 * sizeof(unsigned long long)));
  return VBT_OK;
}
#endif
```

### vbt_amd/csrc/plan_geom.h

```cpp
#pragma once
#include <algorithm>

#include "launchers.h"

namespace vbt {

inline void choose_tile(int OH, int OW, int KK, int S, bool expand, int* TXo, int* TYo, int slots = 64) {
  double best = 1e300;
  for (int TX = 1; TX <= std::min(OW, 64); TX++) {
    int TXp = (TX + 3) & ~3;
    int TY = std::min(OH, slots / TXp);
    if (TY < 1) continue;
    int tiles = ((OW + TX - 1) / TX) * ((OH + TY - 1) / TY);
    int NPh = ((TXp - 1) * S + KK) * ((TY - 1) * S + KK);
    double cost = tiles * ((expand ? 1.0 : 0.35) * NPh + (double)slots);
    if (cost < best) { best = cost; *TXo = TX; *TYo = TY; }
  }
}

inline int fused_tile_lds(const FusedArgs& a, int k, int stride, int TX, int TY, int est, int ppw, int nbp, int e_bytes = -1) {
  const int TXp = (TX + 3) & ~3;
  const int NPh = ((TXp - 1) * stride + k) * ((TY - 1) * stride + k);
  int lds = ((NPh * a.T0S + 15) & ~15) + (e_bytes >= 0 ? e_bytes : ((NPh * est + 15) & ~15)) + ppw * 64 * FB_DST;
  if (!est && a.nchunks == 1 && nbp <= 2) lds += nbp * (4096 + 512);
  return lds;
}

inline int band_lds(const BandArgs& a, bool chained = false) {
  const int NT = (a.Cout + 15) / 16;
  const int t0 = (a.rows + 2) * (a.W + 2) * a.CS, wp = NT * a.KS * 1024 + BD_WP_TAIL;
  return chained ? t0 + wp + BD_WD_CHAIN : t0 + (((a.rows * a.W + 15) >> 4) << 4) * a.CS + wp;
}

}
```

### vbt_amd/csrc/planner.hip

```cpp
#include <algorithm>
#include <cmath>
#include <cstdlib>
#include <functional>
#include <initializer_list>

#include "detector_model.h"
using vbt::v4i;
#include "weight_pack.h"

namespace vbt {

static int conv_kb(const vbt_model* m, const OpRec& op) {
  const bool off = getenv("VBT_NO_KBIAS") != nullptr;
  if (off || (op.type != OP_STEM && op.type != OP_PW && op.type != OP_DW)) return 0;
  const TensorRec& tin = m->tensors[op.inputs[0]];
  const TensorRec& tout = m->tensors[op.output];
  const int8_t* w = (const int8_t*)(m->blob.data() + op.w_off);
  const int32_t* bq = (const int32_t*)(m->blob.data() + op.b_off);
  const bool dw = op.type == OP_DW;
  const int N = tout.c, K = dw ? op.k * op.k : op.k * op.k * tin.c;
  for (int co = 0; co < N; co++) {
    long long sa = 0;
    for (int k = 0; k < K; k++) sa += std::abs((int)(dw ? w[(size_t)k * N + co] : w[(size_t)co * K + k]));
    if (255 * sa + std::llabs((long long)bq[co]) >= (1ll << 22) - 1) return 0;
  }
  return 1;
}


struct NodeSrc { int n = 0; int tensor[3]; int mode[3]; int rs_op[3] = {-1, -1, -1}; int pre_add = -1; int chain = 0; };

static Cost cost_of(const vbt_model* m, std::initializer_list<int> ops, const NodeSrc* ns = nullptr) {
  Cost c;
  for (int oi : ops)
    if (oi >= 0) c += m->op_steps[oi].cost;
  if (ns) c += cost_of(m, {ns->rs_op[0], ns->rs_op[1], ns->rs_op[2], ns->pre_add});
  return c;
}

template <typename Args>
static void fill_node_sources(Args& a, const NodeSrc& ns, const vbt_model* m, int sum_op) {
  a.n_src = ns.n;
  for (int j = 0; j < ns.n; j++) {
    const TensorRec& ts = m->tensors[ns.tensor[j]];
    a.sh[j] = ts.h; a.sw[j] = ts.w; a.smode[j] = ns.mode[j];
    if (ns.mode[j] == 2) { a.spt[j] = m->ops[ns.rs_op[j]].pad_t; a.spl[j] = m->ops[ns.rs_op[j]].pad_l; }
  }
  a.sumq = m->op_steps[sum_op].addq;
  a.chain = 0;
  if (ns.pre_add >= 0) {
    a.chain = ns.chain;
    a.preq = m->op_steps[ns.pre_add].addq;
  }
}

static int make_image_bundle(vbt_model* m, int e_op, int d_op, int p_op, int KSe, ImageBundle* out) {
  const OpRec &eop = m->ops[e_op], &dop = m->ops[d_op], &pop = m->ops[p_op];
  const TensorRec &tin = m->tensors[eop.inputs[0]], &tdin = m->tensors[dop.inputs[0]], &tout = m->tensors[pop.output];
  const int8_t* we = (const int8_t*)(m->blob.data() + eop.w_off);
  const int8_t* wd = (const int8_t*)(m->blob.data() + dop.w_off);
  const int8_t* wpj = (const int8_t*)(m->blob.data() + pop.w_off);
  const int Ce = tdin.c, Cp = (Ce + 63) / 64 * 64, kk = dop.k * dop.k, NB = (tout.c + 63) / 64, nch = Cp / 64;
  std::vector<long> pe, pp;
  pack_weights(we, Ce, tin.c, KSe, nch, nullptr, pe);
  pack_weights(wpj, tout.c, Ce, Cp / 32, NB, nullptr, pp);
  const std::vector<int> be = fold_bias((const int32_t*)(m->blob.data() + eop.b_off), we, Ce, tin.c, tin.zero_point, W_ROWS, Cp);
  const std::vector<int> bd = fold_bias((const int32_t*)(m->blob.data() + dop.b_off), wd, Ce, kk, tdin.zero_point, W_TAPS, Cp);
  const std::vector<float> me = pad_floats((const float*)(m->blob.data() + eop.m_off), Ce, Cp);
  const std::vector<float> md = pad_floats((const float*)(m->blob.data() + dop.m_off), Ce, Cp);
  ImageBundle ib;
  ib.o_be = KSe * 2048; ib.o_me = ib.o_be + 256; ib.o_dw = ib.o_me + 256;
  ib.o_bd = ib.o_dw + ((kk * 64 + 15) & ~15); ib.o_md = ib.o_bd + 256; ib.o_wp = ib.o_md + 256;
  ib.bytes = ib.o_wp + NB * 4096;
  std::vector<unsigned char> rec((size_t)nch * ib.bytes, 0);
  for (int c = 0; c < nch; c++) {
    unsigned char* R = rec.data() + (size_t)c * ib.bytes;
    memcpy(R, pe.data() + (size_t)c * KSe * 4 * 64, (size_t)KSe * 2048);
    memcpy(R + ib.o_be, &be[64 * c], 256);
    memcpy(R + ib.o_me, &me[64 * c], 256);
    memcpy(R + ib.o_bd, &bd[64 * c], 256);
    memcpy(R + ib.o_md, &md[64 * c], 256);
    for (int t = 0; t < kk; t++)
      for (int i = 0; i < 64 && 64 * c + i < Ce; i++) R[ib.o_dw + t * 64 + i] = (unsigned char)wd[(size_t)t * Ce + 64 * c + i];
    for (int nb = 0; nb < NB; nb++)
      for (int k2 = 0; k2 < 2; k2++)
        memcpy(R + ib.o_wp + (size_t)((nb * 2 + k2) * 4) * 512, pp.data() + ((size_t)(nb * (Cp / 32) + 2 * c + k2) * 4) * 64, 4 * 512);
  }
  unsigned char* drec;
  int rc;
  if ((rc = upload(m, rec, &drec))) return rc;
  ib.data = drec;
  *out = ib;
  return VBT_OK;
}

static int make_fused_params(vbt_model* m, int e_op, int d_op, int p_op, Step* sp) {
  Step& s = *sp;
  const FusedArgs& a = s.fa;
  const OpRec &eop = m->ops[e_op], &dop = m->ops[d_op], &pop = m->ops[p_op];
  const TensorRec &tin = m->tensors[eop.inputs[0]], &tdin = m->tensors[dop.inputs[0]], &tdout = m->tensors[dop.output], &tout = m->tensors[pop.output];
  const int8_t* we = (const int8_t*)(m->blob.data() + eop.w_off);
  const int8_t* wd = (const int8_t*)(m->blob.data() + dop.w_off);
  const int8_t* wpj = (const int8_t*)(m->blob.data() + pop.w_off);
  const int Ce = tdin.c, Cp = (Ce + 63) / 64 * 64, kk = dop.k * dop.k, k = dop.k, S = dop.stride;
  if (!(a.KSe == 1 || a.KSe == 2) || s.nbp > 2 || !(k == 3 || k == 5)) return VBT_OK;
  const std::vector<int> be = fold_bias((const int32_t*)(m->blob.data() + eop.b_off), we, Ce, tin.c, tin.zero_point, W_ROWS, Cp);
  const std::vector<float> me = pad_floats((const float*)(m->blob.data() + eop.m_off), Ce, Cp);
  const std::vector<int> bdm = fold_bias((const int32_t*)(m->blob.data() + dop.b_off), wd, Ce, kk, tdin.zero_point, W_TAPS, Cp);
  const std::vector<float> md = pad_floats((const float*)(m->blob.data() + dop.m_off), Ce, Cp);
  const std::vector<int> bp = fold_bias((const int32_t*)(m->blob.data() + pop.b_off), wpj, tout.c, Ce, tdout.zero_point, W_ROWS, s.nbp * 64);
  const std::vector<float> mp = pad_floats((const float*)(m->blob.data() + pop.m_off), tout.c, s.nbp * 64);
  for (int nt3 = 0; nt3 < 2; nt3++) {
    if (nt3 && !a.nch3) continue;
    const int NT = nt3 ? 3 : 4, nch = nt3 ? a.nch3 : a.nchunks;
    std::vector<long> wex;
    if (nt3) wex = pack_expand48(we, Ce, tin.c, a.KSe);
    else pack_weights(we, Ce, tin.c, a.KSe, nch, nullptr, wex);
    const std::vector<int> kmap = nt3 ? kmap48(Ce) : std::vector<int>();
    for (int form = 0; form < 3; form++) {
      FusedLaunch L{k, S, s.nbp, true, true, bool(nt3), false, form != FPF_MATRIX, 0, 0, form == FPF_TOEPLITZ};
      if (form == FPF_TOEPLITZ ? !a.wtz : form == FPF_DIAG64 ? !a.wd64c : false) continue;
      std::vector<long> dwl;
      std::vector<unsigned> dwt;
      for (int tail = 0; tail < 2; tail++) {
        if (tail && !(nt3 ? a.wpt3 : a.wpt)) continue;
        const int ntl = tail ? s.ntl : 0;
        FusedLaunch L2 = L;
        L2.ppw2 = true;
        if (!fused_params_built(L, a.KSe, ntl) && !fused_params_built(L2, a.KSe, ntl)) continue;
        if (dwl.empty() && dwt.empty()) {
          if (form == FPF_DIAG64) dwl = pack_dw64_compact(pack_dw64(wd, Ce, k, Cp / 16), k);
          else if (form == FPF_TOEPLITZ) dwt = pack_expdw2_taps(wd, Ce, 0, Cp / 4, k, S);
          else dwl = pack_dw_diag(wd, Ce, kk, nt3 ? 48 : 64);
        }
        std::vector<v4i> panel;
        if (tail) pack_weights64_tail(wpj, tout.c, Ce, nch, s.nbp, panel, nt3 ? &kmap : nullptr);
        else pack_weights64(wpj, tout.c, Ce, nch, s.nbp, panel, nt3 ? &kmap : nullptr);
        const FusedParamsGeom g = fused_params_geom(NT, a.KSe, form, k, S, s.nbp, ntl);
        const FusedParamsSrc src{wex.data(), be.data(), me.data(), form == FPF_TOEPLITZ ? (const void*)dwt.data() : (const void*)dwl.data(), bdm.data(), md.data(),
                                 panel.data(), nch, bp.data(), mp.data()};
        unsigned char* dev;
        int rc;
        if ((rc = upload(m, pack_fused_chunk_params(g, NT, s.nbp, ntl, nch, src), &dev))) return rc;
        s.cpar[nt3][form][tail] = dev;
      }
    }
  }
  return VBT_OK;
}

static int make_fused(vbt_model* m, int e_op, int d_op, int p_op, int a_op, Step* out, int sum_op = -1, const NodeSrc* ns = nullptr) {
  const OpRec& dop = m->ops[d_op];
  const OpRec& pop = m->ops[p_op];
  const bool expand = e_op >= 0;
  const int in_t = expand ? m->ops[e_op].inputs[0] : dop.inputs[0];
  const TensorRec& tin = m->tensors[in_t];
  const TensorRec& tdin = m->tensors[dop.inputs[0]];
  const TensorRec& tdout = m->tensors[dop.output];
  const TensorRec& tout = m->tensors[pop.output];
  const int Ce = tdin.c, Cp = (Ce + 63) / 64 * 64, kk = dop.k * dop.k;
  const int8_t* wd = (const int8_t*)(m->blob.data() + dop.w_off);
  const int32_t* bqd = (const int32_t*)(m->blob.data() + dop.b_off);
  const int8_t* wpj = (const int8_t*)(m->blob.data() + pop.w_off);
  int rc;
  Step s;
  s.family = expand ? F_MBCONV : (sum_op >= 0 ? F_NODE : F_SEPCONV);
  s.sum_op = sum_op;
  s.op = a_op >= 0 ? a_op : p_op;
  s.e_op = e_op; s.d_op = d_op; s.p_op = p_op; s.a_op = a_op;
  FusedArgs& a = s.fa;
  memset(&a, 0, sizeof(a));
  a.H = tin.h; a.W = tin.w; a.Cin = tin.c; a.OH = tout.h; a.OW = tout.w; a.Cout = tout.c;
  a.pad_t = dop.pad_t; a.pad_l = dop.pad_l;
  choose_tile(tout.h, tout.w, dop.k, dop.stride, expand, &a.TX, &a.TY);
  a.tiles_x = (tout.w + a.TX - 1) / a.TX;
  a.tiles_y = (tout.h + a.TY - 1) / a.TY;
  a.nchunks = Cp / 64;
  a.zx = tin.zero_point;
  const Step& ps = m->op_steps[p_op];
  s.nbp = ps.NB <= 3 ? ps.NB : 5;
  if (expand) {
    const Step& es = m->op_steps[e_op];
    const OpRec& eop = m->ops[e_op];
    a.we = es.wp; a.be = es.bias; a.me = es.mult; a.KSe = es.KS;
    a.ze = tdin.zero_point; a.loe = eop.act_min; a.hie = eop.act_max;
    a.rqe = make_rq(a.ze, a.loe, a.hie, conv_kb(m, eop));
    a.T0S = ((tin.c + 7) & ~7) + 8;
  } else {
    a.T0S = Cp + 16;
  }
  {
    float* dwf; int* dbias; float* dmult;
    if ((rc = upload(m, dw_weights_f32(wd, Ce, kk, Cp), &dwf)) || (rc = upload(m, fold_bias(bqd, wd, Ce, kk, 128 + tdin.zero_point, W_TAPS, Cp), &dbias)) ||
        (rc = upload(m, pad_floats((const float*)(m->blob.data() + dop.m_off), Ce, Cp), &dmult)))
      return rc;
    a.wd = dwf; a.bd = dbias; a.md = dmult;
    long* dwdm; int* dbm;
    if ((rc = upload(m, pack_dw_diag(wd, Ce, kk, 64), &dwdm)) || (rc = upload(m, fold_bias(bqd, wd, Ce, kk, tdin.zero_point, W_TAPS, Cp), &dbm))) return rc;
    a.wdm = dwdm; a.bdm = dbm;
    if (expand && (dop.k == 3 || dop.k == 5)) {
      const std::vector<v4i> w64 = pack_dw64(wd, Ce, dop.k, Cp / 16);
      v4i* d64; long* d64c;
      if ((rc = upload(m, w64, &d64)) || (rc = upload(m, pack_dw64_compact(w64, dop.k), &d64c))) return rc;
      a.wd64 = d64; a.wd64c = d64c;
      if (fused_tpz_built(dop.k, dop.stride, s.nbp, a.KSe, false)) {
        unsigned* dtz;
        if ((rc = upload(m, pack_expdw2_taps(wd, Ce, 0, Cp / 4, dop.k, dop.stride), &dtz))) return rc;
        a.wtz = dtz;
      }
    }
    a.zd = tdout.zero_point; a.lod = dop.act_min; a.hid = dop.act_max;
    a.rqd = make_rq(a.zd, a.lod, a.hid, conv_kb(m, dop));
  }
  {
    std::vector<v4i> wp;
    pack_weights64(wpj, tout.c, Ce, Cp / 64, s.nbp, wp);
    v4i* dwp;
    if ((rc = upload(m, wp, &dwp))) return rc;
    a.wp = dwp; a.bp = ps.bias; a.mp = ps.mult; a.KSp = Cp / 64;
    if (expand && tout.c % 64 != 0 && tout.c % 4 == 0 && s.nbp == (tout.c + 63) / 64) {
      pack_weights64_tail(wpj, tout.c, Ce, Cp / 64, s.nbp, wp);
      if ((rc = upload(m, wp, &dwp))) return rc;
      a.wpt = dwp;
      s.ntl = proj_tail_tiles(tout.c);
    }
    if (expand)
      for (int i = 0; i < d_op; i++) s.block += m->ops[i].type == OP_DW;
    a.zo = tout.zero_point; a.lop = pop.act_min; a.hip = pop.act_max;
    a.rqp = make_rq(a.zo, a.lop, a.hip);
  }
  if (a_op >= 0) {
    a.has_res = 1;
    a.resq = m->op_steps[a_op].addq;
  }
  if (sum_op >= 0) {
    fill_node_sources(a, *ns, m, sum_op);
    for (int j = 0; j < ns->n; j++) s.src_tensor[j] = ns->tensor[j];
  }
  s.lds_bytes = fused_tile_lds(a, dop.k, dop.stride, a.TX, a.TY, expand ? FB_EST : 0, 1, s.nbp);
  s.cost = cost_of(m, {e_op, d_op, p_op, a_op, sum_op}, ns);
  if (expand && Ce % 48 == 0 && Ce % 64 != 0) {
    const int8_t* we = (const int8_t*)(m->blob.data() + m->ops[e_op].w_off);
    const int nch3 = Ce / 48;
    const std::vector<int> kmap = kmap48(Ce);
    std::vector<v4i> wp3;
    pack_weights64(wpj, tout.c, Ce, nch3, s.nbp, wp3, &kmap);
    long *d1, *d2;
    v4i* d3;
    if ((rc = upload(m, pack_expand48(we, Ce, tin.c, a.KSe), &d1)) || (rc = upload(m, pack_dw_diag(wd, Ce, kk, 48), &d2)) || (rc = upload(m, wp3, &d3))) return rc;
    a.we3 = d1; a.wdm3 = d2; a.wp3 = d3; a.nch3 = nch3; a.KSp3 = nch3;
    if (s.ntl) {
      pack_weights64_tail(wpj, tout.c, Ce, nch3, s.nbp, wp3, &kmap);
      if ((rc = upload(m, wp3, &d3))) return rc;
      a.wpt3 = d3;
    }
  }
  if (expand && (rc = make_fused_params(m, e_op, d_op, p_op, &s))) return rc;
  if (expand && tin.h * tin.w <= 400 && tout.h * tout.w <= 400 && (rc = make_image_bundle(m, e_op, d_op, p_op, a.KSe, &s.ib))) return rc;
  *out = s;
  return VBT_OK;
}

static const Alt* tile_alt(const Group& g, int family) {
  for (int i = (int)g.alts.size() - 1; i >= 0; i--)
    if (g.alts[i].steps.size() == 1 && g.alts[i].steps[0].family == family) return &g.alts[i];
  return nullptr;
}
static const Alt* band_alt(const Group& g) {
  for (int i = (int)g.alts.size() - 1; i >= 0; i--)
    if (g.alts[i].steps.size() == 1 && g.alts[i].steps[0].family == F_BAND && g.alts[i].steps[0].members.empty()) return &g.alts[i];
  return nullptr;
}

static bool band_ok(const vbt_model* m, int d_op, int p_op) {
  if (m->flags & VBT_MODEL_NO_BAND) return false;
  if (const char* ns = getenv("VBT_SUBSTREAMS")) if (atoi(ns) > 1) return false;
  const OpRec& d = m->ops[d_op];
  const OpRec& p = m->ops[p_op];
  const TensorRec& ti = m->tensors[d.inputs[0]];
  const TensorRec& to = m->tensors[p.output];
  return d.k == 3 && d.stride == 1 && d.pad_t == 1 && d.pad_l == 1 && ti.c % 8 == 0 && ti.c >= 16 && ti.c <= 128 && to.c <= 128 && to.h == ti.h &&
         to.w == ti.w && ti.w <= 160;
}
static int make_band(vbt_model* m, int d_op, int p_op, int sum_op, const NodeSrc* ns, Step* out) {
  const OpRec& dop = m->ops[d_op];
  const OpRec& pop = m->ops[p_op];
  const TensorRec& tin = m->tensors[dop.inputs[0]];
  const TensorRec& td = m->tensors[dop.output];
  const TensorRec& to = m->tensors[pop.output];
  Step s;
  s.family = F_BAND;
  s.op = p_op;
  s.d_op = d_op;
  s.p_op = p_op;
  s.sum_op = sum_op;
  BandArgs& a = s.bd_args;
  memset(&a, 0, sizeof(a));
  a.H = tin.h; a.W = tin.w; a.Cout = to.c;
  const int C = tin.c;
  a.C = C;
  a.CS = ((C + 15) / 16 | 1) * 16;
  a.NCG = (C + 15) / 16;
  a.KS = (C + 63) / 64;
  static const int band_px_env = getenv("VBT_BAND_PX") ? atoi(getenv("VBT_BAND_PX")) : 0;
  const int band_px = band_px_env > 0 ? band_px_env : (m->max_batch <= 8 ? 64 : 320);
  const int nb = std::max(1, (tin.h * tin.w + band_px - 1) / band_px);
  a.rows = (tin.h + nb - 1) / nb;
  a.nbands = (tin.h + a.rows - 1) / a.rows;
  a.zx4 = (unsigned)(tin.zero_point & 255) * 0x01010101u;
  const int8_t* wd = (const int8_t*)(m->blob.data() + dop.w_off);
  v4i *dpd, *dpp, *dpc = nullptr;
  int* dbd;
  float* dmd;
  int rc;
  if ((rc = upload(m, pack_band_dw(wd, C), &dpd)) || (rc = upload(m, pack_band_pw((const int8_t*)(m->blob.data() + pop.w_off), to.c, C), &dpp)) ||
      (rc = upload(m, fold_bias((const int32_t*)(m->blob.data() + dop.b_off), wd, C, 9, tin.zero_point, W_TAPS, a.NCG * 16), &dbd)) ||
      (rc = upload(m, pad_floats((const float*)(m->blob.data() + dop.m_off), C, a.NCG * 16), &dmd)))
    return rc;
  if (C == 64 && to.c <= 64 && (rc = upload(m, pack_band_pw_chain((const int8_t*)(m->blob.data() + pop.w_off), to.c, C), &dpc))) return rc;
  a.wd = dpd; a.wp = dpp; a.wpc = dpc; a.bd = dbd; a.md = dmd;
  a.bp = m->op_steps[p_op].bias;
  a.mp = m->op_steps[p_op].mult;
  a.rqd = make_rq(td.zero_point, dop.act_min, dop.act_max, conv_kb(m, dop));
  a.rqp = make_rq(to.zero_point, pop.act_min, pop.act_max, conv_kb(m, pop));
  a.x = m->tptr[dop.inputs[0]];
  a.out = m->tptr[pop.output];
  if (sum_op >= 0) {
    fill_node_sources(a, *ns, m, sum_op);
    a.x = nullptr;
    for (int j = 0; j < ns->n; j++) a.src[j] = m->tptr[ns->tensor[j]];
  }
  s.band_tiles = a.nbands;
  s.lds_bytes = band_lds(a);
  std::vector<BandArgs> one{a};
  if ((rc = upload(m, one, &s.d_band))) return rc;
  s.cost = cost_of(m, {d_op, p_op, sum_op}, ns);
  *out = s;
  return VBT_OK;
}

static int batch_heads(vbt_model* m) {
  struct Info { int gi, chain, depth; };
  std::vector<Info> heads;
  std::map<int, std::pair<int, int>> by_tensor;
  int nchains = 0, first = -1;
  for (int gi = 0; gi < (int)m->groups.size(); gi++) {
    const Group& g = m->groups[gi];
    const Alt* fap = tile_alt(g, F_SEPCONV);
    if (!fap) continue;
    const Step& st = fap->steps[0];
    if (m->ops[st.d_op].level < 0) continue;
    int tin = m->ops[st.d_op].inputs[0], tout = m->ops[st.p_op].output;
    auto it = by_tensor.find(tin);
    int chain = it == by_tensor.end() ? nchains++ : it->second.first;
    int depth = it == by_tensor.end() ? 0 : it->second.second + 1;
    by_tensor[tout] = {chain, depth};
    heads.push_back({gi, chain, depth});
    if (first < 0) first = gi;
  }
  if (heads.size() < 2) return VBT_OK;
  int maxd = 0;
  for (auto& h : heads) maxd = std::max(maxd, h.depth);
  auto members_of = [&](int d) {
    std::vector<int> mem;
    for (auto& h : heads)
      if (h.depth == d) mem.push_back(h.gi);
    return mem;
  };
  auto mergeable = [&](const std::vector<int>& mem) {
    if (mem.size() < 2 || mem.size() > 12) return false;
    const Step& s0 = tile_alt(m->groups[mem[0]], F_SEPCONV)->steps[0];
    if (!((s0.nbp == 1 || s0.nbp == 2) && m->ops[s0.d_op].k == 3 && m->ops[s0.d_op].stride == 1)) return false;
    for (int gi : mem) {
      const Step& st = tile_alt(m->groups[gi], F_SEPCONV)->steps[0];
      if (st.nbp != s0.nbp || m->ops[st.d_op].k != 3 || m->ops[st.d_op].stride != 1) return false;
    }
    return true;
  };
  int d0 = maxd + 1;
  while (d0 > 0 && mergeable(members_of(d0 - 1))) d0--;
  if (d0 > maxd) return VBT_OK;
  std::map<int, Group> at;
  std::vector<char> consumed(m->groups.size(), 0);
  for (int d = d0; d <= maxd; d++) {
    std::vector<int> mem = members_of(d);
    const Step& s0 = tile_alt(m->groups[mem[0]], F_SEPCONV)->steps[0];
    Group g;
    Alt unf, each, multi, bandm;
    Step ms, bs;
    bs.family = F_BAND;
    bs.op = s0.op;
    bs.d_op = s0.d_op;
    std::vector<BandArgs> bargs;
    bool all_band = true;
    ms.family = F_MULTI;
    ms.op = s0.op;
    ms.d_op = s0.d_op;
    ms.nbp = s0.nbp;
    std::vector<FusedArgs> hargs;
    int last = 0;
    for (int gi : mem) {
      const Group& src = m->groups[gi];
      for (const Step& st : src.alts[0].steps) unf.steps.push_back(st);
      const Alt* ta = tile_alt(src, F_SEPCONV);
      const Step& fs = ta->steps[0];
      each.steps.push_back(fs);
      for (int t : ta->hidden) { each.hidden.push_back(t); multi.hidden.push_back(t); bandm.hidden.push_back(t); }
      const Alt* ba = band_alt(src);
      if (ba && ba->steps[0].bd_args.n_src == 0) {
        Step b1 = ba->steps[0];
        {
          BandArgs& ha = b1.bd_args;
          const int nbh = std::max(1, (ha.H * ha.W + BD_HEAD_MAXPX - 1) / BD_HEAD_MAXPX);
          ha.rows = (ha.H + nbh - 1) / nbh;
          ha.nbands = (ha.H + ha.rows - 1) / ha.rows;
          b1.band_tiles = ha.nbands;
          b1.lds_bytes = band_lds(ha);
        }
        bs.members.push_back(b1);
        bargs.push_back(b1.bd_args);
        bs.lds_bytes = std::max(bs.lds_bytes, b1.lds_bytes);
        bs.cost += b1.cost;
      } else {
        all_band = false;
      }
      ms.members.push_back(fs);
      ms.lds_bytes = std::max(ms.lds_bytes, fs.lds_bytes);
      ms.cost += fs.cost;
      FusedArgs a = fs.fa;
      a.x = m->tptr[m->ops[fs.d_op].inputs[0]];
      a.out = m->tptr[m->ops[fs.op].output];
      hargs.push_back(a);
      consumed[gi] = 1;
      last = std::max(last, gi);
    }
    int rc = upload(m, hargs, &ms.d_multi);
    if (rc) return rc;
    multi.steps.push_back(ms);
    g.alts.push_back(unf);
    g.alts.push_back(each);
    g.alts.push_back(multi);
    g.chosen = 2;
    if (all_band && bargs.size() <= 12) {
      int rcb = upload(m, bargs, &bs.d_band);
      if (rcb) return rcb;
      bandm.steps.push_back(bs);
      g.alts.push_back(bandm);
      g.chosen = 3;
    }
    at[last] = g;
  }
  std::vector<Group> out;
  for (int gi = 0; gi < (int)m->groups.size(); gi++) {
    if (!consumed[gi]) out.push_back(m->groups[gi]);
    auto it = at.find(gi);
    if (it != at.end()) out.push_back(it->second);
  }
  m->groups.swap(out);
  return VBT_OK;
}

static bool stem_block_ok(const vbt_model* m, int si, const std::vector<int>& consumers) {
  const int no = (int)m->ops.size();
  if (si + 2 >= no) return false;
  const OpRec& st = m->ops[si];
  const OpRec& d = m->ops[si + 1];
  const OpRec& p = m->ops[si + 2];
  if (st.type != OP_STEM || d.type != OP_DW || p.type != OP_PW) return false;
  const TensorRec& ti = m->tensors[st.inputs[0]];
  const TensorRec& ts = m->tensors[st.output];
  const TensorRec& td = m->tensors[d.output];
  const TensorRec& to = m->tensors[p.output];
  return st.k == 3 && st.stride == 2 && ti.c == 3 && ts.c == 32 && ti.w % 4 == 0 && d.inputs[0] == st.output && consumers[st.output] == 1 &&
         d.k == 3 && d.stride == 1 && d.pad_t == 1 && d.pad_l == 1 && td.c == 32 && p.inputs[0] == d.output && consumers[d.output] == 1 &&
         to.c <= 16 && to.c % 4 == 0;
}

static int make_stem_block(vbt_model* m, int si, Step* out) {
  const OpRec& st = m->ops[si];
  const OpRec& d = m->ops[si + 1];
  const OpRec& p = m->ops[si + 2];
  const TensorRec& ti = m->tensors[st.inputs[0]];
  const TensorRec& ts = m->tensors[st.output];
  const TensorRec& td = m->tensors[d.output];
  const TensorRec& to = m->tensors[p.output];
  Step s;
  s.op = si + 2;
  s.family = F_STEMBLK;
  s.e_op = si;
  s.d_op = si + 1;
  s.p_op = si + 2;
  StemBlockArgs& a = s.sb;
  a.frames = nullptr; a.out = nullptr;
  a.H = ti.h; a.W = ti.w; a.SH = ts.h; a.SW = ts.w; a.Cout = to.c;
  a.spad_t = st.pad_t; a.spad_l = st.pad_l;
  a.tiles_x = (ts.w + 15) / 16; a.tiles_y = (ts.h + 15) / 16;
  a.in_pad4 = (unsigned)((ti.zero_point + 128) & 255) * 0x01010101u;
  a.zs4 = (unsigned)(ts.zero_point & 255) * 0x01010101u;
  a.rqs = make_rq(ts.zero_point, st.act_min, st.act_max, conv_kb(m, st));
  a.rqd = make_rq(td.zero_point, d.act_min, d.act_max, conv_kb(m, d));
  a.rqp = make_rq(to.zero_point, p.act_min, p.act_max, conv_kb(m, p));
  int rc;
  {
    const int8_t* w = (const int8_t*)(m->blob.data() + st.w_off);
    long* dws; int* dbs; float* dms;
    if ((rc = upload(m, pack_stem_block_stem(w), &dws)) || (rc = upload(m, fold_bias((const int32_t*)(m->blob.data() + st.b_off), w, 32, 27, ti.zero_point, W_ROWS), &dbs)) ||
        (rc = upload(m, pad_floats((const float*)(m->blob.data() + st.m_off), 32, 32), &dms)))
      return rc;
    a.ws = dws; a.bs = dbs; a.ms = dms;
    v4i* dws64;
    if ((rc = upload(m, pack_stem_block_stem64(w), &dws64))) return rc;
    a.ws64 = dws64;
    a.in_pad4s = a.in_pad4 ^ 0x80808080u;
  }
  const Step& ds = m->op_steps[si + 1];
  a.bdm = ds.bdm; a.mdm = ds.mdm;
  v4i* d64;
  if ((rc = upload(m, pack_dw64((const int8_t*)(m->blob.data() + d.w_off), 32, 3, 2), &d64))) return rc;
  a.wd64 = d64;
  {
    const int8_t* w = (const int8_t*)(m->blob.data() + p.w_off);
    long* dwp; int* dbp; float* dmp;
    if ((rc = upload(m, pack_stem_block_proj(w, to.c), &dwp)) || (rc = upload(m, fold_bias((const int32_t*)(m->blob.data() + p.b_off), w, to.c, 32, td.zero_point, W_ROWS, 16), &dbp)) ||
        (rc = upload(m, pad_floats((const float*)(m->blob.data() + p.m_off), to.c, 16), &dmp)))
      return rc;
    a.wp = dwp; a.bp = dbp; a.mp = dmp;
    long* dwpc;
    if ((rc = upload(m, pack_stem_block_proj_chain(w, to.c), &dwpc))) return rc;
    a.wpc = dwpc;
  }
  s.cost = cost_of(m, {si, si + 1, si + 2});
  *out = s;
  return VBT_OK;
}

struct ExpDwGeom { int nbands, brows, t0_bytes, e_bytes, d_bytes; };
static ExpDwGeom expdw_geom(int H, int W, int OH, int OW, int k, int stride, int pad_t, int pad_l, int T0S, int nbands) {
  ExpDwGeom g;
  g.nbands = nbands;
  g.brows = (OH + nbands - 1) / nbands;
  g.nbands = (OH + g.brows - 1) / g.brows;
  const int PW = std::max((OW - 1) * stride + k, pad_l + W);
  int in_rows = 0;
  for (int b = 0; b < g.nbands; b++) {
    const int oy0 = b * g.brows, oy1 = std::min(oy0 + g.brows, OH);
    const int PHb = (oy1 - oy0 - 1) * stride + k;
    const int lo = std::max(oy0 * stride - pad_t, 0), hi = std::min(oy0 * stride - pad_t + PHb, H);
    in_rows = std::max(in_rows, hi - lo);
  }
  const int PHmax = (g.brows - 1) * stride + k;
  g.t0_bytes = (in_rows * W * T0S + 15) & ~15;
  g.e_bytes = PHmax * PW * XD_EST;
  g.d_bytes = ((g.brows * OW + 15) / 16) * 16 * XD_EST;
  return g;
}
static ExpDwGeom expdw_choose(int H, int W, int OH, int OW, int k, int stride, int pad_t, int pad_l, int T0S) {
  const int budget = 96 * 1024;
  ExpDwGeom g = expdw_geom(H, W, OH, OW, k, stride, pad_t, pad_l, T0S, 1);
  if (H * W <= 400 && OH * OW <= 400 && g.t0_bytes + g.e_bytes + g.d_bytes <= 160 * 1024) return g;
  for (int nb = 2; nb <= OH; nb++) {
    g = expdw_geom(H, W, OH, OW, k, stride, pad_t, pad_l, T0S, nb);
    if (g.t0_bytes + g.e_bytes + g.d_bytes <= budget) return g;
  }
  return g;
}
static bool expdw_ok(const vbt_model* m, int e_op, int d_op) {
  const OpRec& e = m->ops[e_op];
  const OpRec& d = m->ops[d_op];
  const TensorRec& tin = m->tensors[e.inputs[0]];
  const TensorRec& tout = m->tensors[d.output];
  const int KS64 = (tin.c + 63) / 64;
  const bool shape = (d.k == 3 && d.stride == 1) || (d.k == 5 && (d.stride == 1 || d.stride == 2));
  if (!(shape && tin.h * tin.w <= 1024 && tin.c % 8 == 0 && tout.c % 16 == 0 && KS64 >= 2 && KS64 <= 4)) return false;
  const ExpDwGeom g = expdw_choose(tin.h, tin.w, tout.h, tout.w, d.k, d.stride, d.pad_t, d.pad_l, ((tin.c + 15) / 16 | 1) * 16);
  return g.t0_bytes + g.e_bytes + g.d_bytes <= 160 * 1024;
}
static int make_expdw2(vbt_model* m, int e_op, int d_op, Step* s, const std::vector<v4i>& pe, const std::vector<int>& be, const std::vector<float>& me,
                       const std::vector<int>& bd, const std::vector<float>& md);
static int make_expdw(vbt_model* m, int e_op, int d_op, Step* out) {
  const OpRec& eop = m->ops[e_op];
  const OpRec& dop = m->ops[d_op];
  const TensorRec& tin = m->tensors[eop.inputs[0]];
  const TensorRec& te = m->tensors[eop.output];
  const TensorRec& td = m->tensors[dop.output];
  Step s;
  s.family = F_EXPDW;
  s.op = d_op;
  s.e_op = e_op;
  s.d_op = d_op;
  ExpDwArgs& a = s.xd;
  memset(&a, 0, sizeof(a));
  a.H = tin.h; a.W = tin.w; a.Cin = tin.c; a.OH = td.h; a.OW = td.w; a.Ce = te.c;
  a.pad_t = dop.pad_t; a.pad_l = dop.pad_l;
  a.PH = std::max((a.OH - 1) * dop.stride + dop.k, a.pad_t + a.H);
  a.PW = std::max((a.OW - 1) * dop.stride + dop.k, a.pad_l + a.W);
  const int K = tin.c, Ce = te.c, nch = (Ce + 63) / 64, kk = dop.k * dop.k;
  a.T0S = ((tin.c + 15) / 16 | 1) * 16;
  a.nchunks = nch;
  a.cpw = 1;
  const ExpDwGeom geo = expdw_choose(a.H, a.W, a.OH, a.OW, dop.k, dop.stride, a.pad_t, a.pad_l, a.T0S);
  a.nbands = geo.nbands; a.brows = geo.brows; a.t0_bytes = geo.t0_bytes; a.e_bytes = geo.e_bytes;
  const int8_t* we = (const int8_t*)(m->blob.data() + eop.w_off);
  const int8_t* wd = (const int8_t*)(m->blob.data() + dop.w_off);
  const std::vector<v4i> pe = pack_expdw_expand(we, Ce, K);
  const std::vector<int> be = fold_bias((const int32_t*)(m->blob.data() + eop.b_off), we, Ce, K, tin.zero_point, W_ROWS, nch * 64);
  const std::vector<int> bd = fold_bias((const int32_t*)(m->blob.data() + dop.b_off), wd, Ce, kk, te.zero_point, W_TAPS, nch * 64);
  const std::vector<float> me = pad_floats((const float*)(m->blob.data() + eop.m_off), Ce, nch * 64);
  const std::vector<float> md = pad_floats((const float*)(m->blob.data() + dop.m_off), Ce, nch * 64);
  v4i* dpe;
  long* dpd;
  int *dbe, *dbd;
  float *dme, *dmd;
  int rc;
  if ((rc = upload(m, pe, &dpe)) || (rc = upload(m, pack_expdw_taps(wd, Ce, kk), &dpd)) || (rc = upload(m, be, &dbe)) || (rc = upload(m, bd, &dbd)) ||
      (rc = upload(m, me, &dme)) || (rc = upload(m, md, &dmd)))
    return rc;
  a.we = dpe; a.wdc = dpd; a.be = dbe; a.bd = dbd; a.me = dme; a.md = dmd;
  a.rqe = make_rq(te.zero_point, eop.act_min, eop.act_max, conv_kb(m, eop));
  a.rqd = make_rq(td.zero_point, dop.act_min, dop.act_max, conv_kb(m, dop));
  a.zeb = (unsigned)(te.zero_point & 255) * 0x01010101u;
  s.lds_bytes = geo.t0_bytes + geo.e_bytes + geo.d_bytes;
  s.cost = cost_of(m, {e_op, d_op});
  if ((rc = make_expdw2(m, e_op, d_op, &s, pe, be, me, bd, md))) return rc;
// ... 588 lines not shown
```

### vbt_amd/csrc/weight_pack.h

```cpp
#pragma once
#include <algorithm>
#include <cstdint>
#include <cstring>
#include <vector>

#include "fused_params_geom.h"

inline void pack_weights(const int8_t* w, int N, int K, int KS, int NB, const std::vector<int>* kmap, std::vector<long>& out) {
  out.assign((size_t)NB * KS * 4 * 64, 0);
  int8_t* o = (int8_t*)out.data();
  for (int nb = 0; nb < NB; nb++)
    for (int ks = 0; ks < KS; ks++)
      for (int t = 0; t < 4; t++)
        for (int lane = 0; lane < 64; lane++) {
          int i = lane & 15, g = lane >> 4;
          int co = 64 * nb + 16 * (i >> 2) + 4 * t + (i & 3);
          for (int j = 0; j < 8; j++) {
            int kp = 32 * ks + 8 * g + j;
            int k = kmap ? (kp < (int)kmap->size() ? (*kmap)[kp] : -1) : (kp < K ? kp : -1);
            int8_t v = (co < N && k >= 0) ? w[(size_t)co * K + k] : 0;
            o[((((size_t)(nb * KS + ks) * 4 + t) * 64 + lane) * 8) + j] = v;
          }
        }
}

inline void pack_weights64(const int8_t* w, int N, int K, int KS, int NB, std::vector<v4i>& out, const std::vector<int>* kmap = nullptr) {
  out.assign((size_t)NB * KS * 4 * 64, (v4i){0, 0, 0, 0});
  int8_t* o = (int8_t*)out.data();
  for (int nb = 0; nb < NB; nb++)
    for (int ks = 0; ks < KS; ks++)
      for (int t = 0; t < 4; t++)
        for (int lane = 0; lane < 64; lane++) {
          const int i = lane & 15, g = lane >> 4, co = 64 * nb + 16 * (i >> 2) + 4 * t + (i & 3);
          for (int j = 0; j < 16; j++) {
            const int kp = 64 * ks + 16 * g + j;
            const int k = kmap ? (kp < (int)kmap->size() ? (*kmap)[kp] : -1) : (kp < K ? kp : -1);
            o[((((size_t)(nb * KS + ks) * 4 + t) * 64 + lane) * 16) + j] = (co < N && k >= 0) ? w[(size_t)co * K + k] : 0;
          }
        }
}

inline int proj_tail_tiles(int N) { return ((N % 64) + 15) / 16; }
inline void pack_weights64_tail(const int8_t* w, int N, int K, int KS, int NB, std::vector<v4i>& out, const std::vector<int>* kmap = nullptr) {
  if (N % 64 == 0 || NB != (N + 63) / 64) { pack_weights64(w, N, K, KS, NB, out, kmap); return; }
  const int NTL = proj_tail_tiles(N), nbl = NB - 1;
  std::vector<v4i> full;
  pack_weights64(w, 64 * nbl, K, KS, nbl, full, kmap);
  out.assign((size_t)nbl * KS * 4 * 64 + (size_t)KS * NTL * 64, (v4i){0, 0, 0, 0});
  std::copy(full.begin(), full.end(), out.begin());
  int8_t* o = (int8_t*)(out.data() + (size_t)nbl * KS * 4 * 64);
  for (int ks = 0; ks < KS; ks++)
    for (int t = 0; t < NTL; t++)
      for (int lane = 0; lane < 64; lane++) {
        const int i = lane & 15, g = lane >> 4, co = 64 * nbl + 16 * t + i;
        for (int j = 0; j < 16; j++) {
          const int kp = 64 * ks + 16 * g + j;
          const int k = kmap ? (kp < (int)kmap->size() ? (*kmap)[kp] : -1) : (kp < K ? kp : -1);
          o[(((size_t)(ks * NTL + t) * 64 + lane) * 16) + j] = (co < N && k >= 0) ? w[(size_t)co * K + k] : 0;
        }
      }
}

enum WLayout { W_ROWS, W_TAPS };
inline std::vector<int> fold_bias(const int32_t* bq, const int8_t* w, int n, int K, int zp, WLayout layout, int padded = 0) {
  std::vector<int> out(std::max(n, padded), 0);
  for (int c = 0; c < n; c++) {
    long sw = 0;
    for (int k = 0; k < K; k++) sw += layout == W_ROWS ? w[(size_t)c * K + k] : w[(size_t)k * n + c];
    out[c] = (int)((long)bq[c] - (long)zp * sw);
  }
  return out;
}
template <typename T>
inline std::vector<float> pad_floats(const T* v, int n, int padded) {
  std::vector<float> out(std::max(n, padded), 0.0f);
  for (int c = 0; c < n; c++) out[c] = (float)v[c];
  return out;
}
inline std::vector<float> dw_weights_f32(const int8_t* w, int C, int kk, int Cp) {
  std::vector<float> out((size_t)kk * Cp, 0.0f);
  for (int t = 0; t < kk; t++)
    for (int c = 0; c < C; c++) out[(size_t)t * Cp + c] = (float)w[(size_t)t * C + c];
  return out;
}

inline std::vector<long> pack_dw_diag(const int8_t* w, int C, int kk, int group_channels) {
  const int NCG = group_channels / 16, nch = (C + group_channels - 1) / group_channels, KT = (kk + 1) / 2;
  std::vector<long> out((size_t)nch * NCG * KT * 64, 0);
  int8_t* o = (int8_t*)out.data();
  for (int ch = 0; ch < nch; ch++)
    for (int cg = 0; cg < NCG; cg++)
      for (int mi = 0; mi < KT; mi++)
        for (int lane = 0; lane < 64; lane++) {
          const int i = lane & 15, g = lane >> 4, c = group_channels * ch + 16 * cg + i, tap = 2 * mi + (g >> 1);
          for (int j = 0; j < 8; j++)
            o[((((size_t)(ch * NCG + cg) * KT + mi) * 64 + lane) * 8) + j] = (tap < kk && 8 * (g & 1) + j == i && c < C) ? w[(size_t)tap * C + c] : 0;
        }
  return out;
}

inline std::vector<v4i> pack_dw64(const int8_t* w, int C, int k, int nq) {
  const int K64 = k == 3 ? 3 : 7;
  std::vector<v4i> out((size_t)nq * K64 * 64, (v4i){0, 0, 0, 0});
  int8_t* o = (int8_t*)out.data();
  for (int q = 0; q < nq; q++)
    for (int mi = 0; mi < K64; mi++)
      for (int lane = 0; lane < 64; lane++) {
        const int i = lane & 15, g = lane >> 4, c = 16 * q + i;
        int tap = -1;
        if (k == 3) tap = g < 3 ? mi * 3 + g : -1;
        else if (mi < 5) tap = mi * 5 + g;
        else if (mi == 5) tap = g * 5 + 4;
        else tap = g == 0 ? 24 : -1;
        if (tap >= 0 && c < C) o[(((size_t)q * K64 + mi) * 64 + lane) * 16 + i] = w[(size_t)tap * C + c];
      }
  return out;
}
inline std::vector<long> pack_dw64_compact(const std::vector<v4i>& w64, int k) {
  const int K64 = k == 3 ? 3 : 7, nq = (int)(w64.size() / ((size_t)K64 * 64));
  std::vector<long> out((size_t)nq * 64, 0);
  const int8_t* o = (const int8_t*)w64.data();
  int8_t* oc = (int8_t*)out.data();
  for (int q = 0; q < nq; q++)
    for (int mi = 0; mi < K64; mi++)
      for (int lane = 0; lane < 64; lane++)
        oc[((size_t)q * 64 + lane) * 8 + mi] = o[(((size_t)q * K64 + mi) * 64 + lane) * 16 + (lane & 15)];
  return out;
}

inline std::vector<long> pack_expand48(const int8_t* w, int Ce, int K, int KS) {
  const int nch3 = Ce / 48;
  std::vector<long> out((size_t)nch3 * KS * 3 * 64, 0);
  int8_t* o = (int8_t*)out.data();
  for (int c = 0; c < nch3; c++)
    for (int ks = 0; ks < KS; ks++)
      for (int t = 0; t < 3; t++)
        for (int lane = 0; lane < 64; lane++) {
          const int i = lane & 15, kg = lane >> 4, co = 48 * c + 12 * (i >> 2) + 4 * t + (i & 3);
          for (int j = 0; j < 8; j++) {
            const int k = 32 * ks + 8 * kg + j;
            o[((((size_t)(c * KS + ks) * 3 + t) * 64 + lane) * 8) + j] = k < K ? w[(size_t)co * K + k] : 0;
          }
        }
  return out;
}
inline std::vector<int> kmap48(int Ce) {
  std::vector<int> kmap((size_t)(Ce / 48) * 64, -1);
  for (int c = 0; c < Ce / 48; c++)
    for (int q = 0; q < 48; q++) kmap[(size_t)c * 64 + q] = 48 * c + q;
  return kmap;
}

inline std::vector<v4i> pack_band_dw(const int8_t* w, int C) {
  const int NCG = (C + 15) / 16;
  std::vector<v4i> out((size_t)NCG * 3 * 64, (v4i){0, 0, 0, 0});
  int8_t* o = (int8_t*)out.data();
  for (int cg = 0; cg < NCG; cg++)
    for (int mi = 0; mi < 3; mi++)
      for (int lane = 0; lane < 64; lane++) {
        const int i = lane & 15, g = lane >> 4, ch = 16 * cg + i, tap = 4 * mi + g;
        for (int j = 0; j < 16; j++) o[(((size_t)(cg * 3 + mi) * 64 + lane) * 16) + j] = (tap < 9 && j == i && ch < C) ? w[(size_t)tap * C + ch] : 0;
      }
  return out;
}
inline std::vector<v4i> pack_band_pw(const int8_t* w, int N, int C) {
  const int NT = (N + 15) / 16, KS = (C + 63) / 64;
  std::vector<v4i> out((size_t)NT * KS * 64, (v4i){0, 0, 0, 0});
  int8_t* o = (int8_t*)out.data();
  for (int t = 0; t < NT; t++)
    for (int ks = 0; ks < KS; ks++)
      for (int lane = 0; lane < 64; lane++) {
        const int i = lane & 15, g = lane >> 4, co = 16 * t + i;
        for (int j = 0; j < 16; j++) {
          const int k = 64 * ks + 16 * g + j;
          o[((((size_t)t * KS + ks) * 64 + lane) * 16) + j] = (co < N && k < C) ? w[(size_t)co * C + k] : 0;
        }
      }
  return out;
}
inline std::vector<v4i> pack_band_pw_chain(const int8_t* w, int N, int C) {
  const int NT = (N + 15) / 16;
  std::vector<v4i> out((size_t)NT * 64, (v4i){0, 0, 0, 0});
  int8_t* o = (int8_t*)out.data();
  for (int t = 0; t < NT; t++)
    for (int lane = 0; lane < 64; lane++) {
      const int i = lane & 15, g = lane >> 4, co = 16 * t + i;
      for (int cg = 0; cg < 4; cg++)
        for (int j = 0; j < 4; j++) {
          const int k = 16 * cg + 4 * g + j;
          o[((size_t)t * 64 + lane) * 16 + 4 * cg + j] = (co < N && k < C) ? w[(size_t)co * C + k] : 0;
        }
    }
  return out;
}

inline std::vector<int> stem_kmap() {
  std::vector<int> kmap(32, -1);
  for (int g = 0; g < 3; g++)
    for (int j = 0; j < 8; j++) kmap[8 * g + j] = (g * 3 + j / 3) * 3 + j % 3;
  for (int j = 0; j < 3; j++) kmap[24 + j] = (j * 3 + 2) * 3 + 2;
  return kmap;
}
inline std::vector<long> pack_stem_block_stem(const int8_t* w) {
  std::vector<long> out(2 * 64, 0);
  int8_t* o = (int8_t*)out.data();
  for (int t = 0; t < 2; t++)
    for (int lane = 0; lane < 64; lane++) {
      const int i = lane & 15, kg = lane >> 4, co = 8 * (i >> 2) + 4 * t + (i & 3);
      for (int j = 0; j < 8; j++) {
        const int f = kg < 3 ? kg * 9 + j : (j < 3 ? j * 9 + 8 : -1);
        o[((size_t)t * 64 + lane) * 8 + j] = f >= 0 ? w[(size_t)co * 27 + f] : 0;
      }
    }
  return out;
}
inline std::vector<long> pack_stem_block_proj(const int8_t* w, int N) {
  std::vector<long> out(64, 0);
  int8_t* o = (int8_t*)out.data();
  for (int lane = 0; lane < 64; lane++) {
    const int i = lane & 15, kg = lane >> 4;
    for (int j = 0; j < 8; j++) o[(size_t)lane * 8 + j] = i < N ? w[(size_t)i * 32 + 8 * kg + j] : 0;
  }
  return out;
}
inline std::vector<v4i> pack_stem_block_stem64(const int8_t* w) {
  std::vector<v4i> out(2 * 64, (v4i){0, 0, 0, 0});
  int8_t* o = (int8_t*)out.data();
  for (int t = 0; t < 2; t++)
    for (int lane = 0; lane < 64; lane++) {
      const int i = lane & 15, g = lane >> 4, co = 8 * (i >> 2) + 4 * t + (i & 3);
      for (int j = 0; j < 9 && g < 3; j++) o[((size_t)t * 64 + lane) * 16 + j] = w[(size_t)co * 27 + g * 9 + j];
    }
  return out;
}
inline std::vector<long> pack_stem_block_proj_chain(const int8_t* w, int N) {
  std::vector<long> out(64, 0);
  int8_t* o = (int8_t*)out.data();
  for (int lane = 0; lane < 64; lane++) {
    const int i = lane & 15, g = lane >> 4;
    for (int cg = 0; cg < 2; cg++)
      for (int j = 0; j < 4; j++) o[(size_t)lane * 8 + 4 * cg + j] = i < N ? w[(size_t)i * 32 + 16 * cg + 4 * g + j] : 0;
  }
  return out;
}

inline std::vector<v4i> pack_expdw_expand(const int8_t* w, int Ce, int K) {
  const int nch = (Ce + 63) / 64, KS = (K + 63) / 64;
  std::vector<v4i> out((size_t)nch * KS * 4 * 64, (v4i){0, 0, 0, 0});
  int8_t* o = (int8_t*)out.data();
  for (int c = 0; c < nch; c++)
    for (int ks = 0; ks < KS; ks++)
      for (int t = 0; t < 4; t++)
        for (int lane = 0; lane < 64; lane++) {
          const int i = lane & 15, g = lane >> 4, ch = 64 * c + 16 * t + i;
          for (int j = 0; j < 16; j++) {
            const int k = 64 * ks + 16 * g + j;
            o[((((size_t)(c * KS + ks) * 4 + t) * 64 + lane) * 16) + j] = (ch < Ce && k < K) ? w[(size_t)ch * K + k] : 0;
          }
        }
  return out;
}
inline std::vector<long> pack_expdw_taps(const int8_t* w, int Ce, int kk) {
  const int nch = (Ce + 63) / 64, KT = (kk + 3) / 4;
  std::vector<long> out((size_t)nch * 4 * 64, 0);
  int8_t* o = (int8_t*)out.data();
  for (int c = 0; c < nch; c++)
    for (int cg = 0; cg < 4; cg++)
      for (int mi = 0; mi < KT; mi++)
        for (int lane = 0; lane < 64; lane++) {
          const int i = lane & 15, g = lane >> 4, ch = 64 * c + 16 * cg + i, tap = 4 * mi + g;
          o[(((size_t)(c * 4 + cg)) * 64 + lane) * 8 + mi] = (tap < kk && ch < Ce) ? w[(size_t)tap * Ce + ch] : 0;
        }
  return out;
}
inline std::vector<unsigned> pack_expdw2_taps(const int8_t* w, int Ce, int base, int nq, int k, int S) {
  const int KT2 = (S * (S - 1) + k + 1) / 2;
  std::vector<unsigned> out((size_t)nq * KT2 * 64, 0);
  for (int q = 0; q < nq; q++)
    for (int mi = 0; mi < KT2; mi++)
      for (int lane = 0; lane < 64; lane++) {
        const int i = lane & 15, g = lane >> 4, qq = i >> 2, cc = i & 3, ch = base + 4 * q + cc;
        const int dy = S == 2 ? qq >> 1 : 0, dx = S == 2 ? qq & 1 : qq;
        const int ty = 2 * mi + (g >> 1) - S * dy;
        unsigned w4 = 0;
        for (int j = 0; j < 4; j++) {
          const int tx = 4 * (g & 1) + j - S * dx;
          if (ty >= 0 && ty < k && tx >= 0 && tx < k && ch < Ce) w4 |= (unsigned)(uint8_t)w[(size_t)(ty * k + tx) * Ce + ch] << (8 * j);
        }
        out[((size_t)q * KT2 + mi) * 64 + lane] = w4;
      }
  return out;
}

struct FusedParamsSrc {
  const long* we; const int* be; const float* me;
  const void* wdw; const int* bdm; const float* md;
  const v4i* wproj; int KSp;
  const int* bp; const float* mp;
};
inline size_t fused_chunk_params_bytes(const FusedParamsGeom& g, int nch) { return (size_t)nch * g.chunk + g.pb; }
inline std::vector<unsigned char> pack_fused_chunk_params(const FusedParamsGeom& g, int NT, int NBP, int NTL, int nch, const FusedParamsSrc& s) {
  std::vector<unsigned char> out(fused_chunk_params_bytes(g, nch), 0);
  const int CH = 16 * NT, NBW = NTL ? NBP - 1 : NBP;
  for (int c = 0; c < nch; c++) {
    unsigned char* R = out.data() + (size_t)c * g.chunk;
    memcpy(R, (const unsigned char*)s.we + (size_t)c * g.o_be, g.o_be);
    memcpy(R + g.o_be, s.be + c * CH, 4 * CH);
    memcpy(R + g.o_me, s.me + c * CH, 4 * CH);
    R += g.pe;
    memcpy(R, (const unsigned char*)s.wdw + (size_t)c * g.o_bd, g.o_bd);
    memcpy(R + g.o_bd, s.bdm + c * CH, 4 * CH);
    memcpy(R + g.o_md, s.md + c * CH, 4 * CH);
    R += g.pd;
    for (int nb = 0; nb < NBW; nb++) memcpy(R + nb * 4096, s.wproj + ((size_t)(nb * s.KSp + c) * 4) * 64, 4096);
    if (NTL) memcpy(R + NBW * 4096, s.wproj + ((size_t)NBW * s.KSp * 4 + (size_t)c * NTL) * 64, NTL * 1024);
  }
  unsigned char* T = out.data() + (size_t)nch * g.chunk;
  memcpy(T, s.bp, NBP * 256);
  memcpy(T + NBP * 256, s.mp, NBP * 256);
  return out;
}
```

Before: 135,600.

## Pack chained depthwise taps compactly and tag global pointers with address space

The chained band kernel now stages only one packed dword of depthwise taps per lane in shared memory, 1 KB instead of 12 KB of diagonal operands, and rebuilds the diagonal MFMA operands in registers with diag_operand. This cuts LDS footprint and staging traffic, which may raise occupancy. In exchange it adds ALU work per channel group. Separately, global loads across band, node and postprocess kernels go through address_space(1) pointers and a gload helper so the compiler emits global rather than flat memory instructions.

```diff
diff --git a/vbt_amd/csrc/band_block.h b/vbt_amd/csrc/band_block.h
--- a/vbt_amd/csrc/band_block.h
+++ b/vbt_amd/csrc/band_block.h
@@ -1,6 +1,7 @@
 #pragma once
 #include <type_traits>
 
+#include "band_geom.h"
 #include "fused_block.h"
 
 namespace vbt {
@@ -12,8 +13,6 @@
 constexpr int BD_LIT = 3;
 constexpr int BD_LIT_NODE = 1;
 constexpr int BD_LIT_NODE_WIDE = 3;
-constexpr int BD_WP_TAIL = 1024;
-constexpr int BD_WD_CHAIN = 12 * 1024 + 512;
 
 #ifdef VBT_BD_PROF
 #define BD_STAMP(k) do { if (threadIdx.x == 0) a.prof[(long)blockIdx.x * 8 + (k)] = __builtin_amdgcn_s_memtime(); } while (0)
@@ -29,6 +28,7 @@
   int NCG, KS;
   unsigned zx4;
   const v4i* wd;
+  const unsigned* wdt;
   const int* bd;
   const float* md;
   Rq rqd;
@@ -46,15 +46,53 @@
 #endif
 };
 
-__device__ __forceinline__ unsigned band_source4(const BandArgs& a, int j, long b, int iy, int ix, int cd, bool up2) {
+struct BandView {
+  gptr<const int8_t> x;
+  gptr<int8_t> out;
+  int H, W, Cout, rows, nbands, C, CS, NCG, KS;
+  unsigned zx4;
+  gptr<const v4i> wd;
+  gptr<const unsigned> wdt;
+  gptr<const int> bd;
+  gptr<const float> md;
+  Rq rqd;
+  gptr<const v4i> wp, wpc;
+  gptr<const int> bp;
+  gptr<const float> mp;
+  Rq rqp;
+  int n_src, chain;
+  gptr<const int8_t> src[3];
+  int sh[3], sw[3], smode[3], spt[3], spl[3];
+  AddQ sumq, preq;
+#ifdef VBT_BD_PROF
+  gptr<unsigned long long> prof;
+#endif
+  __device__ __forceinline__ explicit BandView(const BandArgs& a)
+      : x(gptr_cast<const int8_t>(a.x)), out(gptr_cast<int8_t>(a.out)), H(a.H), W(a.W), Cout(a.Cout), rows(a.rows), nbands(a.nbands), C(a.C), CS(a.CS),
+        NCG(a.NCG), KS(a.KS), zx4(a.zx4), wd(gptr_cast<const v4i>(a.wd)), wdt(gptr_cast<const unsigned>(a.wdt)), bd(gptr_cast<const int>(a.bd)),
+        md(gptr_cast<const float>(a.md)), rqd(a.rqd),
+        wp(gptr_cast<const v4i>(a.wp)), wpc(gptr_cast<const v4i>(a.wpc)), bp(gptr_cast<const int>(a.bp)), mp(gptr_cast<const float>(a.mp)), rqp(a.rqp),
+        n_src(a.n_src), chain(a.chain), sumq(a.sumq), preq(a.preq) {
+#pragma unroll
+    for (int j = 0; j < 3; j++) {
+      src[j] = gptr_cast<const int8_t>(a.src[j]);
+      sh[j] = a.sh[j]; sw[j] = a.sw[j]; smode[j] = a.smode[j]; spt[j] = a.spt[j]; spl[j] = a.spl[j];
+    }
+#ifdef VBT_BD_PROF
+    prof = gptr_cast<unsigned long long>(a.prof);
+#endif
+  }
+};
+
+__device__ __forceinline__ unsigned band_source4(const BandView& a, int j, long b, int iy, int ix, int cd, bool up2) {
   const int C = a.C;
-  const int8_t* sb = a.src[j] + b * (long)a.sh[j] * a.sw[j] * C + 4 * cd;
-  if (a.smode[j] == 0) return *(const unsigned*)(sb + (iy * a.sw[j] + ix) * C);
+  const gptr<const int8_t> sb = a.src[j] + b * (long)a.sh[j] * a.sw[j] * C + 4 * cd;
+  if (a.smode[j] == 0) return *gptr_cast<const unsigned>(sb + (iy * a.sw[j] + ix) * C);
   if (a.smode[j] == 1) {
     int yy, xx;
     if (up2) { yy = iy >> 1; xx = ix >> 1; }
     else { yy = (iy * a.sh[j]) / a.H; xx = (ix * a.sw[j]) / a.W; }
-    return *(const unsigned*)(sb + (yy * a.sw[j] + xx) * C);
+    return *gptr_cast<const unsigned>(sb + (yy * a.sw[j] + xx) * C);
   }
   unsigned lo = 0u, hi = 0u;
 #pragma unroll
@@ -63,7 +101,7 @@
 #pragma unroll
     for (int kx = 0; kx < 3; kx++) {
       const int xx = ix * 2 + kx - a.spl[j], xc = min(max(xx, 0), a.sw[j] - 1);
-      unsigned t = *(const unsigned*)(sb + (yc * a.sw[j] + xc) * C);
+      unsigned t = *gptr_cast<const unsigned>(sb + (yc * a.sw[j] + xc) * C);
       t = (yy == yc && xx == xc) ? (t ^ 0x80808080u) : 0u;
       lo = pk_max_u16(lo, t & 0x00FF00FFu);
       hi = pk_max_u16(hi, (t >> 8) & 0x00FF00FFu);
@@ -72,15 +110,15 @@
   return (lo | (hi << 8)) ^ 0x80808080u;
 }
 
-__device__ __forceinline__ uint4 band_source16(const BandArgs& a, int j, long b, int iy, int ix, int sg, bool up2) {
+__device__ __forceinline__ uint4 band_source16(const BandView& a, int j, long b, int iy, int ix, int sg, bool up2) {
   const int C = a.C;
-  const int8_t* sb = a.src[j] + b * (long)a.sh[j] * a.sw[j] * C + 16 * sg;
-  if (a.smode[j] == 0) return *(const uint4*)(sb + (iy * a.sw[j] + ix) * C);
+  const gptr<const int8_t> sb = a.src[j] + b * (long)a.sh[j] * a.sw[j] * C + 16 * sg;
+  if (a.smode[j] == 0) return gload<uint4>(sb + (iy * a.sw[j] + ix) * C);
   if (a.smode[j] == 1) {
     int yy, xx;
     if (up2) { yy = iy >> 1; xx = ix >> 1; }
     else { yy = (iy * a.sh[j]) / a.H; xx = (ix * a.sw[j]) / a.W; }
-    return *(const uint4*)(sb + (yy * a.sw[j] + xx) * C);
+    return gload<uint4>(sb + (yy * a.sw[j] + xx) * C);
   }
   unsigned lo[4] = {0u, 0u, 0u, 0u}, hi[4] = {0u, 0u, 0u, 0u};
 #pragma unroll
@@ -89,7 +127,7 @@
 #pragma unroll
     for (int kx = 0; kx < 3; kx++) {
       const int xx = ix * 2 + kx - a.spl[j], xc = min(max(xx, 0), a.sw[j] - 1);
-      const uint4 t4 = *(const uint4*)(sb + (yc * a.sw[j] + xc) * C);
+      const uint4 t4 = gload<uint4>(sb + (yc * a.sw[j] + xc) * C);
       const bool in = yy == yc && xx == xc;
       const unsigned tt[4] = {t4.x, t4.y, t4.z, t4.w};
 #pragma unroll
@@ -105,7 +143,7 @@
 }
 
 template <int NW, int CT, bool NODES = true, bool CHAIN = false>
-__device__ __forceinline__ void sepconv_band_body(const BandArgs& a, int local, unsigned char* bd_smem) {
+__device__ __forceinline__ void sepconv_band_body(const BandView& a, int local, unsigned char* bd_smem) {
   constexpr int nwaves = NW, nthreads = 64 * NW;
   static_assert(!CHAIN || CT == 64, "the chained form is built for 64-channel maps");
   constexpr bool C64 = CT == 64, CK = CT != 0;
@@ -124,15 +162,16 @@
   unsigned char* WB = WP + NT * KS * 1024;
   BD_STAMP(0);
 
-  const v4i* wpg = CHAIN ? a.wpc : a.wp;
+  const gptr<const v4i> wpg = CHAIN ? a.wpc : a.wp;
   for (int i = tid; i < NT * KS * 64; i += nthreads) *(v4i*)(WP + 16 * i) = wpg[i];
   if constexpr (CHAIN) {
-    for (int i = tid; i < 12 * 64; i += nthreads) *(v4i*)(WB + BD_WP_TAIL + 16 * i) = a.wd[i];
-    if (tid >= 64 && tid < 80) *(uint4*)(WB + BD_WP_TAIL + 12 * 1024 + 16 * (tid - 64)) = *(const uint4*)((const unsigned char*)a.bd + 16 * (tid - 64));
-    else if (tid >= 96 && tid < 112) *(uint4*)(WB + BD_WP_TAIL + 12 * 1024 + 256 + 16 * (tid - 96)) = *(const uint4*)((const unsigned char*)a.md + 16 * (tid - 96));
-  }
-  if (tid < 4 * NT) *(uint4*)(WB + 16 * tid) = *(const uint4*)((const unsigned char*)a.bp + 16 * tid);
-  else if (tid >= 32 && tid < 32 + 4 * NT) *(uint4*)(WB + 512 + 16 * (tid - 32)) = *(const uint4*)((const unsigned char*)a.mp + 16 * (tid - 32));
+    static_assert(nthreads >= 128 + BD_WD_TAPS / 16, "one 16-byte piece of the taps per thread, behind the bias / multiplier threads");
+    if (tid >= 128 && tid < 128 + BD_WD_TAPS / 16) *(uint4*)(WB + BD_WP_TAIL + 16 * (tid - 128)) = gload<uint4>(a.wdt + 4 * (tid - 128));
+    if (tid >= 64 && tid < 80) *(uint4*)(WB + BD_WP_TAIL + BD_WD_TAPS + 16 * (tid - 64)) = gload<uint4>(a.bd + 4 * (tid - 64));
+    else if (tid >= 96 && tid < 112) *(uint4*)(WB + BD_WP_TAIL + BD_WD_TAPS + 256 + 16 * (tid - 96)) = gload<uint4>(a.md + 4 * (tid - 96));
+  }
+  if (tid < 4 * NT) *(uint4*)(WB + 16 * tid) = gload<uint4>(a.bp + 4 * tid);
+  else if (tid >= 32 && tid < 32 + 4 * NT) *(uint4*)(WB + 512 + 16 * (tid - 32)) = gload<uint4>(a.mp + 4 * (tid - 32));
   const float rcp_pw = frcp(PW);
   if (NODES && a.n_src > 0) {
     const bool up2[3] = {a.H == 2 * a.sh[0] && a.W == 2 * a.sw[0], a.H == 2 * a.sh[1] && a.W == 2 * a.sw[1], a.H == 2 * a.sh[2] && a.W == 2 * a.sw[2]};
@@ -202,7 +241,7 @@
     }
     }
   } else {
-    const int8_t* xb = a.x + b * (long)a.H * a.W * C;
+    const gptr<const int8_t> xb = a.x + b * (long)a.H * a.W * C;
     if constexpr (C64) {
       const uint4 z4 = make_uint4(a.zx4, a.zx4, a.zx4, a.zx4);
       const int total = NPh * 4;
@@ -217,7 +256,7 @@
           const int iy = y0 + hy - 1, ix = hx - 1;
           pofs[k] = i < total ? p * 80 + 16 * sg : -1;
           v[k] = z4;
-          if (i < total && iy >= 0 && iy < a.H && ix >= 0 && ix < a.W) v[k] = *(const uint4*)(xb + (iy * a.W + ix) * 64 + 16 * sg);
+          if (i < total && iy >= 0 && iy < a.H && ix >= 0 && ix < a.W) v[k] = gload<uint4>(xb + (iy * a.W + ix) * 64 + 16 * sg);
         }
 #pragma unroll
         for (int k = 0; k < BD_LIT; k++)
@@ -240,7 +279,7 @@
           const int iy = y0 + hy - 1, ix = hx - 1;
           pofs[k] = i < total ? p * CS + 16 * sg : -1;
           v[k] = z4;
-          if (i < total && sg < nreal && iy >= 0 && iy < a.H && ix >= 0 && ix < a.W) v[k] = *(const uint4*)(xb + (iy * a.W + ix) * C + 16 * sg);
+          if (i < total && sg < nreal && iy >= 0 && iy < a.H && ix >= 0 && ix < a.W) v[k] = gload<uint4>(xb + (iy * a.W + ix) * C + 16 * sg);
         }
 #pragma unroll
         for (int k = 0; k < BD_LIT; k++)
@@ -255,7 +294,7 @@
       const int hy = fdiv_small(p, rcp_pw), hx = p - hy * PW;
       const int iy = y0 + hy - 1, ix = hx - 1;
       uint2 v = z2;
-      if (sg < ng && iy >= 0 && iy < a.H && ix >= 0 && ix < a.W) v = *(const uint2*)(xb + (iy * a.W + ix) * C + 8 * sg);
+      if (sg < ng && iy >= 0 && iy < a.H && ix >= 0 && ix < a.W) v = gload<uint2>(xb + (iy * a.W + ix) * C + 8 * sg);
       *(uint2*)(T0 + p * CS + 8 * sg) = v;
     }
     }
@@ -270,10 +309,10 @@
   const float rcp_w = frcp(a.W);
   if constexpr (CHAIN) {
     const unsigned char* WD = WB + BD_WP_TAIL;
-    const unsigned char* WDB = WD + 12 * 1024;
+    const unsigned char* WDB = WD + BD_WD_TAPS;
     __syncthreads();
     BD_STAMP(1);
-    int8_t* ob = a.out + ((b * a.H + y0) * (long)a.W) * a.Cout + 4 * g;
+    const gptr<int8_t> ob = a.out + ((b * a.H + y0) * (long)a.W) * a.Cout + 4 * g;
     const bool dword_out = (a.Cout & 3) == 0;
     auto chain = [&](auto fd_c, auto u_c, int pg0) {
       constexpr int U = decltype(u_c)::value, FULL = decltype(fd_c)::value;
@@ -291,8 +330,9 @@
 #pragma unroll
         for (int cg = 0; cg < 4; cg++) {
           v4i wdv[3], bv[U][3], acc[U];
-#pragma unroll
-          for (int m = 0; m < 3; m++) wdv[m] = *(const v4i*)(WD + ((cg * 3 + m) * 64 + lane) * 16);
+          const unsigned wt = *(const unsigned*)(WD + (cg * 64 + lane) * 4);
+#pragma unroll
+          for (int m = 0; m < 3; m++) wdv[m] = diag_operand((wt >> (8 * m)) & 255u, r);
           const int4 bq = *(const int4*)(WDB + 64 * cg + 16 * g);
           const float4 mu = *(const float4*)(WDB + 256 + 64 * cg + 16 * g);
 #pragma unroll
@@ -324,8 +364,8 @@
           for (int u = 0; u < U; u++) {
             const unsigned d = rq_pack_b<FULL>(acc[u], mm, a.rqp);
             if (slot[u] < NPo && c0 < a.Cout) {
-              int8_t* o = ob + (long)slot[u] * a.Cout + 16 * t;
-              if (dword_out) *(unsigned*)o = d;
+              const gptr<int8_t> o = ob + (long)slot[u] * a.Cout + 16 * t;
+              if (dword_out) *gptr_cast<unsigned>(o) = d;
               else
                 for (int j = 0; j < 4; j++)
                   if (c0 + j < a.Cout) o[j] = (int8_t)(d >> (8 * j));
@@ -346,8 +386,8 @@
   v4i wdv[3];
 #pragma unroll
   for (int m = 0; m < 3; m++) wdv[m] = a.wd[(cg * 3 + m) * 64 + lane];
-  const int4 bq = *(const int4*)(a.bd + 16 * cg + 4 * g);
-  const float4 mu = *(const float4*)(a.md + 16 * cg + 4 * g);
+  const int4 bq = gload<int4>(a.bd + 16 * cg + 4 * g);
+  const float4 mu = gload<float4>(a.md + 16 * cg + 4 * g);
   __syncthreads();
   BD_STAMP(1);
   if (sub < nsub) {
@@ -392,8 +432,8 @@
     const int c0 = 16 * t + 4 * g;
     const unsigned d = rq_pack_b(acc, mm, a.rqp);
     if (slot < NPo && c0 < a.Cout) {
-      int8_t* o = a.out + ((b * a.H + y0) * (long)a.W + slot) * a.Cout + c0;
-      if ((a.Cout & 3) == 0) *(unsigned*)o = d;
+      const gptr<int8_t> o = a.out + ((b * a.H + y0) * (long)a.W + slot) * a.Cout + c0;
+      if ((a.Cout & 3) == 0) *gptr_cast<unsigned>(o) = d;
       else
         for (int j = 0; j < 4; j++)
           if (c0 + j < a.Cout) o[j] = (int8_t)(d >> (8 * j));
@@ -404,7 +444,7 @@
     const v4i wv = *(const v4i*)(WP + (t * 64 + lane) * 16);
     const int4 bb = *(const int4*)(WB + 4 * c0);
     const float4 mm = *(const float4*)(WB + 512 + 4 * c0);
-    int8_t* ob = a.out + ((b * a.H + y0) * (long)a.W) * a.Cout + c0;
+    const gptr<int8_t> ob = a.out + ((b * a.H + y0) * (long)a.W) * a.Cout + c0;
     auto p_units = [&](auto full_c, auto u_c, int pg0) {
       constexpr int U = decltype(u_c)::value, FULL = decltype(full_c)::value;
       v4i dv[U], acc[U];
@@ -416,7 +456,7 @@
       for (int u = 0; u < U; u++) {
         const int slot = (pg0 + u * (nwaves / 4)) * 16 + r;
         const unsigned d = rq_pack_b<FULL>(acc[u], mm, a.rqp);
-        if (slot < NPo) *(unsigned*)(ob + (long)slot * a.Cout) = d;
+        if (slot < NPo) *gptr_cast<unsigned>(ob + (long)slot * a.Cout) = d;
       }
     };
     auto p_walk = [&](auto full_c) {
@@ -487,39 +527,39 @@
 __global__ __launch_bounds__(64 * BD_HEAD_WAVES) void sepconv_band_kernel(const BandArgs* __restrict__ probs, MultiTiles mt) {
   extern __shared__ __attribute__((aligned(16))) unsigned char bd_smem_dyn[];
   const int pi = band_problem(mt);
-  sepconv_band_body<BD_HEAD_WAVES, 64, false>(probs[pi], (int)blockIdx.x - mt.start[pi], bd_smem_dyn);
+  sepconv_band_body<BD_HEAD_WAVES, 64, false>(BandView(probs[pi]), (int)blockIdx.x - mt.start[pi], bd_smem_dyn);
 }
 __global__ __launch_bounds__(64 * BD_HEAD_WAVES_WIDE, 2) void sepconv_band_wide_kernel(const BandArgs* __restrict__ probs, MultiTiles mt) {
   extern __shared__ __attribute__((aligned(16))) unsigned char bd_smem_dyn[];
   const int pi = band_problem(mt);
-  sepconv_band_body<BD_HEAD_WAVES_WIDE, 0, false>(probs[pi], (int)blockIdx.x - mt.start[pi], bd_smem_dyn);
+  sepconv_band_body<BD_HEAD_WAVES_WIDE, 0, false>(BandView(probs[pi]), (int)blockIdx.x - mt.start[pi], bd_smem_dyn);
 }
 __global__ __launch_bounds__(64 * BD_HEAD_WAVES_WIDE, 2) void sepconv_band_c112_kernel(const BandArgs* __restrict__ probs, MultiTiles mt) {
   extern __shared__ __attribute__((aligned(16))) unsigned char bd_smem_dyn[];
   const int pi = band_problem(mt);
-  sepconv_band_body<BD_HEAD_WAVES_WIDE, 112, false>(probs[pi], (int)blockIdx.x - mt.start[pi], bd_smem_dyn);
+  sepconv_band_body<BD_HEAD_WAVES_WIDE, 112, false>(BandView(probs[pi]), (int)blockIdx.x - mt.start[pi], bd_smem_dyn);
 }
 __global__ __launch_bounds__(64 * BD_HEAD_WAVES) __attribute__((amdgpu_waves_per_eu(6))) void sepconv_band_chain_kernel(const BandArgs* __restrict__ probs, MultiTiles mt) {
   extern __shared__ __attribute__((aligned(16))) unsigned char bd_smem_dyn[];
   const int pi = band_problem(mt);
-  sepconv_band_body<BD_HEAD_WAVES, 64, false, true>(probs[pi], (int)blockIdx.x - mt.start[pi], bd_smem_dyn);
+  sepconv_band_body<BD_HEAD_WAVES, 64, false, true>(BandView(probs[pi]), (int)blockIdx.x - mt.start[pi], bd_smem_dyn);
 }
 __global__ __launch_bounds__(BD_THREADS) void sepconv_band_one_kernel(BandArgs a) {
   extern __shared__ __attribute__((aligned(16))) unsigned char bd_smem_dyn[];
-  sepconv_band_body<BD_WAVES, 64>(a, (int)blockIdx.x, bd_smem_dyn);
+  sepconv_band_body<BD_WAVES, 64>(BandView(a), (int)blockIdx.x, bd_smem_dyn);
 }
 __global__ __launch_bounds__(BD_THREADS) void sepconv_band_one_chain_kernel(BandArgs a) {
   extern __shared__ __attribute__((aligned(16))) unsigned char bd_smem_dyn[];
-  sepconv_band_body<BD_WAVES, 64, true, true>(a, (int)blockIdx.x, bd_smem_dyn);
+  sepconv_band_body<BD_WAVES, 64, true, true>(BandView(a), (int)blockIdx.x, bd_smem_dyn);
 }
 __global__ __launch_bounds__(BD_THREADS) void sepconv_band_one_wide_kernel(BandArgs a) {
   extern __shared__ __attribute__((aligned(16))) unsigned char bd_smem_dyn[];
-  sepconv_band_body<BD_WAVES, 0>(a, (int)blockIdx.x, bd_smem_dyn);
+  sepconv_band_body<BD_WAVES, 0>(BandView(a), (int)blockIdx.x, bd_smem_dyn);
 }
 __global__ __launch_bounds__(BD_THREADS) void sepconv_band_one_c112_kernel(BandArgs a) {
   extern __shared__ __attribute__((aligned(16))) unsigned char bd_smem_dyn[];
-  sepconv_band_body<BD_WAVES, 112>(a, (int)blockIdx.x, bd_smem_dyn);
-}
-#endif
-
-}
+  sepconv_band_body<BD_WAVES, 112>(BandView(a), (int)blockIdx.x, bd_smem_dyn);
+}
+#endif
+
+}
diff --git a/vbt_amd/csrc/band_geom.h b/vbt_amd/csrc/band_geom.h
--- /dev/null
+++ b/vbt_amd/csrc/band_geom.h
@@ -0,0 +1,11 @@
+#pragma once
+
+constexpr int BD_WP_TAIL = 1024;
+constexpr int BD_WD_TAPS = 4 * 64 * 4;
+constexpr int BD_WD_CHAIN = BD_WD_TAPS + 512;
+
+inline int band_lds_bytes(int rows, int W, int CS, int Cout, int KS, bool chained) {
+  const int NT = (Cout + 15) / 16;
+  const int t0 = (rows + 2) * (W + 2) * CS, wp = NT * KS * 1024 + BD_WP_TAIL;
+  return chained ? t0 + wp + BD_WD_CHAIN : t0 + (((rows * W + 15) >> 4) << 4) * CS + wp;
+}
diff --git a/vbt_amd/csrc/dev_common.h b/vbt_amd/csrc/dev_common.h
--- a/vbt_amd/csrc/dev_common.h
+++ b/vbt_amd/csrc/dev_common.h
@@ -4,6 +4,20 @@
 namespace vbt {
 
 typedef int v4i __attribute__((ext_vector_type(4)));
+
+template <class T>
+using gptr = T __attribute__((address_space(1)))*;
+template <class T, class P>
+__device__ __forceinline__ gptr<T> gptr_cast(P p) { return (gptr<T>)p; }
+template <class T, class P>
+__device__ __forceinline__ T gload(P p) {
+  static_assert(sizeof(T) == 8 || sizeof(T) == 16, "gload: 8- or 16-byte types");
+  typedef unsigned raw_t __attribute__((ext_vector_type(sizeof(T) / 4)));
+  const raw_t v = *gptr_cast<const raw_t>(p);
+  T r;
+  __builtin_memcpy(&r, &v, sizeof(T));
+  return r;
+}
 
 __device__ __forceinline__ int requant(int acc, float mult, int zp, int lo, int hi) {
   float t = (float)acc * mult;
diff --git a/vbt_amd/csrc/fused_block.h b/vbt_amd/csrc/fused_block.h
--- a/vbt_amd/csrc/fused_block.h
+++ b/vbt_amd/csrc/fused_block.h
@@ -147,15 +147,15 @@
 #pragma unroll
         for (int j = 0; j < 3; j++) {
           if (j < a.n_src) {
-            const int8_t* sb = a.src[j] + b * (long)a.sh[j] * a.sw[j] * a.Cin + 4 * cd;
+            const gptr<const int8_t> sb = gptr_cast<const int8_t>(a.src[j]) + b * (long)a.sh[j] * a.sw[j] * a.Cin + 4 * cd;
             unsigned u;
             if (a.smode[j] == 0) {
-              u = *(const unsigned*)(sb + ((long)iy * a.sw[j] + ix) * a.Cin);
+              u = *gptr_cast<const unsigned>(sb + ((long)iy * a.sw[j] + ix) * a.Cin);
             } else if (a.smode[j] == 1) {
               int yy, xx;
               if (up2[j]) { yy = iy >> 1; xx = ix >> 1; }
               else { yy = (iy * a.sh[j]) / a.H; xx = (ix * a.sw[j]) / a.W; }
-              u = *(const unsigned*)(sb + ((long)yy * a.sw[j] + xx) * a.Cin);
+              u = *gptr_cast<const unsigned>(sb + ((long)yy * a.sw[j] + xx) * a.Cin);
             } else {
               unsigned tv[9];
 #pragma unroll
@@ -166,7 +166,7 @@
                 for (int kx = 0; kx < 3; kx++) {
                   const int xx = ix * 2 + kx - a.spl[j];
                   const int xc = min(max(xx, 0), a.sw[j] - 1);
-                  const unsigned t = *(const unsigned*)(sb + ((long)yc * a.sw[j] + xc) * a.Cin);
+                  const unsigned t = *gptr_cast<const unsigned>(sb + ((long)yc * a.sw[j] + xc) * a.Cin);
                   tv[ky * 3 + kx] = (yy == yc && xx == xc) ? (t ^ 0x80808080u) : 0u;
                 }
               }
diff --git a/vbt_amd/csrc/k_postprocess.hip b/vbt_amd/csrc/k_postprocess.hip
--- a/vbt_amd/csrc/k_postprocess.hip
+++ b/vbt_amd/csrc/k_postprocess.hip
@@ -60,26 +60,26 @@
   const int n4 = (A + 3) >> 2;
   const int b1 = p.base[1], b2 = p.base[2], b3 = p.base[3], b4 = p.base[4];
   auto level_of = [&](int a) -> int { return (a >= b1) + (a >= b2) + (a >= b3) + (a >= b4); };
-  const unsigned char *pc0, *pb0;
+  gptr<const unsigned char> pc0, pb0;
   long ce1, ce2, ce3, ce4, be1, be2, be3, be4;
   {
     auto cbias = [&](int l) { return (long)p.cls[l] + (b * (long)(p.base[l + 1] - p.base[l]) - p.base[l]) * (long)p.C; };
     auto bbias = [&](int l) { return (long)p.box[l] + (b * (long)(p.base[l + 1] - p.base[l]) - p.base[l]) * 4; };
-    pc0 = (const unsigned char*)cbias(0); pb0 = (const unsigned char*)bbias(0);
+    pc0 = gptr_cast<const unsigned char>(cbias(0)); pb0 = gptr_cast<const unsigned char>(bbias(0));
     ce1 = cbias(1) - cbias(0); ce2 = cbias(2) - cbias(1); ce3 = cbias(3) - cbias(2); ce4 = cbias(4) - cbias(3);
     be1 = bbias(1) - bbias(0); be2 = bbias(2) - bbias(1); be3 = bbias(3) - bbias(2); be4 = bbias(4) - bbias(3);
   }
-  auto cls_ptr = [&](int a) -> const unsigned char* {
+  auto cls_ptr = [&](int a) -> gptr<const unsigned char> {
     long o = (long)a * p.C;
     o += a >= b1 ? ce1 : 0l; o += a >= b2 ? ce2 : 0l; o += a >= b3 ? ce3 : 0l; o += a >= b4 ? ce4 : 0l;
     return pc0 + o;
   };
-  auto box_ptr = [&](int a) -> const unsigned char* {
+  auto box_ptr = [&](int a) -> gptr<const unsigned char> {
     long o = 4l * a;
     o += a >= b1 ? be1 : 0l; o += a >= b2 ? be2 : 0l; o += a >= b3 ? be3 : 0l; o += a >= b4 ? be4 : 0l;
     return pb0 + o;
   };
-  auto whole = [&](int i, const unsigned char* src) -> bool {
+  auto whole = [&](int i, gptr<const unsigned char> src) -> bool {
     const int a = 4 * i;
     return level_of(a) == level_of(a + 3) && a + 3 < A && (((unsigned long)src) & 3ul) == 0;
   };
@@ -93,12 +93,12 @@
     unsigned w[PS];
 #pragma unroll
     for (int k = 0; k < PS; k++)
-      w[k] = *(const unsigned*)((unsigned long)cls_ptr(4 * min(tid + NT * k, n4 - 1)) & ~3ul);
+      w[k] = *gptr_cast<const unsigned>((unsigned long)cls_ptr(4 * min(tid + NT * k, n4 - 1)) & ~3ul);
 #pragma unroll
     for (int k = 0; k < PS; k++)
       if (tid + NT * k < n4) ((unsigned*)cb)[tid + NT * k] = w[k];
 #pragma unroll 1
-    for (int i = tid + NT * PS; i < n4; i += NT) ((unsigned*)cb)[i] = *(const unsigned*)((unsigned long)cls_ptr(4 * i) & ~3ul);
+    for (int i = tid + NT * PS; i < n4; i += NT) ((unsigned*)cb)[i] = *gptr_cast<const unsigned>((unsigned long)cls_ptr(4 * i) & ~3ul);
 #pragma unroll 1
     for (int i = tid; i < n4; i += NT)
       if (!whole(i, cls_ptr(4 * i))) ((unsigned*)cb)[i] = patch(i);
@@ -108,7 +108,7 @@
 #pragma unroll
       for (int e = 0; e < 4; e++) {
         const int a = min(4 * i + e, A - 1);
-        const signed char* src = (const signed char*)cls_ptr(a);
+        const gptr<const signed char> src = gptr_cast<const signed char>(cls_ptr(a));
         int best = src[0];
         for (int c = 1; c < p.C; c++) best = max(best, (int)src[c]);
         w |= ((unsigned)best & 255u) << (8 * e);
@@ -123,19 +123,19 @@
         const unsigned m1 = pk_max_u16(w1 & 0x00FF00FFu, (w1 >> 8) & 0x00FF00FFu);
         return ((m0 & 0xFFu) | ((m0 >> 8) & 0xFF00u) | ((m1 & 0xFFu) << 16) | ((m1 << 8) & 0xFF000000u)) ^ HB;
       };
-      auto whole2 = [&](int i, const unsigned char* src) -> bool {
+      auto whole2 = [&](int i, gptr<const unsigned char> src) -> bool {
         const int a = 4 * i;
         return level_of(a) == level_of(a + 3) && a + 3 < A && (((unsigned long)src) & 7ul) == 0;
       };
       uint2 w[PS];
 #pragma unroll
       for (int k = 0; k < PS; k++)
-        w[k] = *(const uint2*)((unsigned long)cls_ptr(4 * min(tid + NT * k, n4 - 1)) & ~7ul);
+        w[k] = gload<uint2>((unsigned long)cls_ptr(4 * min(tid + NT * k, n4 - 1)) & ~7ul);
 #pragma unroll
       for (int k = 0; k < PS; k++)
         if (tid + NT * k < n4) ((unsigned*)cb)[tid + NT * k] = pair_max(w[k]);
 #pragma unroll 1
-      for (int i = tid + NT * PS; i < n4; i += NT) ((unsigned*)cb)[i] = pair_max(*(const uint2*)((unsigned long)cls_ptr(4 * i) & ~7ul));
+      for (int i = tid + NT * PS; i < n4; i += NT) ((unsigned*)cb)[i] = pair_max(gload<uint2>((unsigned long)cls_ptr(4 * i) & ~7ul));
 #pragma unroll 1
       for (int i = tid; i < n4; i += NT)
         if (!whole2(i, cls_ptr(4 * i))) ((unsigned*)cb)[i] = best4(i);
@@ -345,7 +345,7 @@
     auto decode = [&](unsigned key, float& sc) -> float4 {
       const int a = (int)(key & 0xFFFFu);
       const int q = 127 - (int)(key >> 16);
-      const unsigned bq = *(const unsigned*)box_ptr(a);
+      const unsigned bq = *gptr_cast<const unsigned>(box_ptr(a));
       const float4 an = *(const float4*)(p.anchors + (long)a * 4);
       const float yc = (float)(s_dq[(int)((bq & 255u) ^ 128u)] * (double)an.z + (double)an.x);
       const float xc = (float)(s_dq[(int)(((bq >> 8) & 255u) ^ 128u)] * (double)an.w + (double)an.y);
@@ -407,7 +407,7 @@
             scores[b * p.max_det + nsel] = ss;
             int cls_id = 0;
             if (p.C > 1) {
-              const unsigned char* src = cls_ptr(sel_anchor);
+              const gptr<const unsigned char> src = cls_ptr(sel_anchor);
               int best = -128;
               for (int c = 0; c < p.C; c++) {
                 const int r = (int)s_rank[(int)(src[c] ^ 128u)];
diff --git a/vbt_amd/csrc/plan_geom.h b/vbt_amd/csrc/plan_geom.h
--- a/vbt_amd/csrc/plan_geom.h
+++ b/vbt_amd/csrc/plan_geom.h
@@ -27,9 +27,7 @@
 }
 
 inline int band_lds(const BandArgs& a, bool chained = false) {
-  const int NT = (a.Cout + 15) / 16;
-  const int t0 = (a.rows + 2) * (a.W + 2) * a.CS, wp = NT * a.KS * 1024 + BD_WP_TAIL;
-  return chained ? t0 + wp + BD_WD_CHAIN : t0 + (((a.rows * a.W + 15) >> 4) << 4) * a.CS + wp;
+  return band_lds_bytes(a.rows, a.W, a.CS, a.Cout, a.KS, chained);
 }
 
 }
diff --git a/vbt_amd/csrc/planner.hip b/vbt_amd/csrc/planner.hip
--- a/vbt_amd/csrc/planner.hip
+++ b/vbt_amd/csrc/planner.hip
@@ -310,6 +310,7 @@
   a.zx4 = (unsigned)(tin.zero_point & 255) * 0x01010101u;
   const int8_t* wd = (const int8_t*)(m->blob.data() + dop.w_off);
   v4i *dpd, *dpp, *dpc = nullptr;
+  unsigned* dpt = nullptr;
   int* dbd;
   float* dmd;
   int rc;
@@ -317,8 +318,10 @@
       (rc = upload(m, fold_bias((const int32_t*)(m->blob.data() + dop.b_off), wd, C, 9, tin.zero_point, W_TAPS, a.NCG * 16), &dbd)) ||
       (rc = upload(m, pad_floats((const float*)(m->blob.data() + dop.m_off), C, a.NCG * 16), &dmd)))
     return rc;
-  if (C == 64 && to.c <= 64 && (rc = upload(m, pack_band_pw_chain((const int8_t*)(m->blob.data() + pop.w_off), to.c, C), &dpc))) return rc;
-  a.wd = dpd; a.wp = dpp; a.wpc = dpc; a.bd = dbd; a.md = dmd;
+  if (C == 64 && to.c <= 64 &&
+      ((rc = upload(m, pack_band_pw_chain((const int8_t*)(m->blob.data() + pop.w_off), to.c, C), &dpc)) || (rc = upload(m, pack_band_dw_taps(wd, C), &dpt))))
+    return rc;
+  a.wd = dpd; a.wdt = dpt; a.wp = dpp; a.wpc = dpc; a.bd = dbd; a.md = dmd;
   a.bp = m->op_steps[p_op].bias;
   a.mp = m->op_steps[p_op].mult;
   a.rqd = make_rq(td.zero_point, dop.act_min, dop.act_max, conv_kb(m, dop));
diff --git a/vbt_amd/csrc/weight_pack.h b/vbt_amd/csrc/weight_pack.h
--- a/vbt_amd/csrc/weight_pack.h
+++ b/vbt_amd/csrc/weight_pack.h
@@ -161,6 +161,19 @@
         const int i = lane & 15, g = lane >> 4, ch = 16 * cg + i, tap = 4 * mi + g;
         for (int j = 0; j < 16; j++) o[(((size_t)(cg * 3 + mi) * 64 + lane) * 16) + j] = (tap < 9 && j == i && ch < C) ? w[(size_t)tap * C + ch] : 0;
       }
+  return out;
+}
+inline std::vector<unsigned> pack_band_dw_taps(const int8_t* w, int C) {
+  const int NCG = (C + 15) / 16;
+  std::vector<unsigned> out((size_t)NCG * 64, 0u);
+  for (int cg = 0; cg < NCG; cg++)
+    for (int lane = 0; lane < 64; lane++) {
+      const int i = lane & 15, g = lane >> 4, ch = 16 * cg + i;
+      for (int mi = 0; mi < 3; mi++) {
+        const int tap = 4 * mi + g;
+        if (tap < 9 && ch < C) out[(size_t)cg * 64 + lane] |= (unsigned)(uint8_t)w[(size_t)tap * C + ch] << (8 * mi);
+      }
+    }
   return out;
 }
 inline std::vector<v4i> pack_band_pw(const int8_t* w, int N, int C) {
```

After: 136,700 (median of 6 runs). No clear change (+0.8%).
